# kowallus/mbgc

Measured on AMD Instinct MI355X. Metric: input Gbases/s (compress hot path, -m1: match-finding + stream emission), higher is better.
Workload: dtype u8

## Files before the change

include/mbgc_swsem.h:

```cpp
#ifndef MBGC_SWSEM_H
#define MBGC_SWSEM_H
#include <stddef.h>
#include <stdint.h>

#ifdef __cplusplus
extern "C" {
#endif

#define SWSEM_NO_LOCK   UINT64_MAX
#define SWSEM_SKIPPED   UINT64_MAX

#define SWSEM_OK         0
#define SWSEM_EINVAL    -1
#define SWSEM_ENOMEM    -2
#define SWSEM_EHIP      -3
#define SWSEM_ELOCK     -4
#define SWSEM_ENODEV    -5

typedef struct swsem swsem_t;

typedef struct {
    uint64_t posSrcText, length, posDestText;
} swsem_match_t;

const char *swsem_last_error(void);
int swsem_device_count(void);
int swsem_device_numa_node(int device);

int swsem_create(swsem_t **out, uint64_t maxRefLength, int L, int k1, int k2, int skipMargin, int device);
void swsem_destroy(swsem_t *h);
int swsem_set_stream(swsem_t *h, void *hip_stream);
int swsem_synchronize(swsem_t *h);

void swsem_disable_sliding_window(swsem_t *h);
void swsem_set_sliding_window_size(swsem_t *h, int factor);
void swsem_disable_circular_buffer(swsem_t *h);
uint64_t swsem_get_ref_length(const swsem_t *h);
uint64_t swsem_get_loading_position(const swsem_t *h);
uint64_t swsem_get_loaded_ref_length(const swsem_t *h);
uint64_t swsem_get_max_ref_length(const swsem_t *h);
uint64_t swsem_get_sliding_window_size(const swsem_t *h);
uint64_t swsem_get_dropped_bytes(const swsem_t *h);
void swsem_set_position(swsem_t *h, uint64_t refPos, int reachedRefLengthCount);
uint64_t swsem_acquire_lock(swsem_t *h);
int swsem_release_lock(swsem_t *h, uint64_t lockValue);
int swsem_get_K(const swsem_t *h);
uint32_t swsem_get_hash_size(const swsem_t *h);

int swsem_load_ref(swsem_t *h, const uint8_t *text, uint64_t len, int loadRC, int addSep, int sep);
int swsem_load_ref_dev(swsem_t *h, const uint8_t *text_dev, uint64_t len, int loadRC, int addSep, int sep);
int swsem_load_separator(swsem_t *h, int sep);
int swsem_finalize_targets(swsem_t *h, int n, const uint8_t *const *ext_dev, const uint64_t *ext_len, int addSep, int sep,
                           int lazySeparator, const uint64_t *lockPos, uint64_t *loadedAfter);
int swsem_revcomp_dev(swsem_t *h, const uint8_t *src_dev, uint64_t n, uint8_t *dst_dev);

int swsem_match(swsem_t *h, const uint8_t *query, uint64_t len, uint32_t minMatchLength, uint64_t lockPos,
                const swsem_match_t **matches, uint64_t *nmatches);

int swsem_match_batch_dev(swsem_t *h, const uint8_t *queries_dev, const uint64_t *offsets, int n,
                          uint32_t minMatchLength, const uint64_t *lockPos);
int swsem_batch_counts(swsem_t *h, uint64_t *nmatches );
int swsem_batch_matches(swsem_t *h, int contig, swsem_match_t *out, uint64_t cap);
int swsem_batch_fingerprint(swsem_t *h, uint64_t *fp, uint64_t *total_matches, uint64_t *total_length);

typedef struct {
    int enableExtensionsWithMismatches;
    int mismatchesWithExclusion;
    int lazyDecompressionSupport;
    int enable40bitReference;
    int frugal64bitLenEncoding;
    int gapDepthOffsetEncoding;
    int gapDepthMismatchesEncoding;
    uint64_t gapBreakingMatchMinLength;
    int mmsMatchBonus, mmsMismatchPenalty, mmsMismatchesScoreThreshold, mmsMismatchesInitialScore;
    int allowedTargetsOutrunForDissimilarContigs;
    uint64_t minimalLengthForDissimilarContigs;
    int unmatchedFractionFactorTweakForDissimilarContigs;
} swsem_emit_params_t;
void swsem_emit_params_default(swsem_emit_params_t *p, int mode );

enum { SWSEM_LIT = 0, SWSEM_OFF = 1, SWSEM_OFF5 = 2, SWSEM_LEN = 3, SWSEM_GAP = 4, SWSEM_FLAGS = 5, SWSEM_NSTREAMS = 6 };

typedef struct {
    const uint8_t *data[SWSEM_NSTREAMS];
    uint64_t size[SWSEM_NSTREAMS];
    uint64_t unmatchedChars;
    uint64_t extensionsMatchedChars, extensionsMismatches, totalMatched, removedGapBreakingMatches;
    uint64_t nmatches;
} swsem_streams_t;

int swsem_emit(swsem_t *h, const swsem_emit_params_t *p, int contig, uint64_t lockPos,
               int unmatchedFractionFactor, int64_t processedTargetsCount, int64_t targetIdx,
               const uint64_t *refExtLoadedPos, uint64_t nLoaded, swsem_streams_t *out);

int swsem_emit_batch(swsem_t *h, const swsem_emit_params_t *p, int n, const int *contigIdx, const uint64_t *lockPos,
                     const int *unmatchedFractionFactor, const int64_t *processedTargetsCount, const int64_t *targetIdx,
                     const uint64_t *refExtLoadedPos, uint64_t nLoaded);
int swsem_emit_batch_begin(swsem_t *h, const swsem_emit_params_t *p, int n, const int *contigIdx, const uint64_t *lockPos,
                           const int *unmatchedFractionFactor, const int64_t *processedTargetsCount, const int64_t *targetIdx,
                           const uint64_t *refExtLoadedPos, uint64_t nLoaded);
typedef struct {
    int ntargets;
    const uint8_t *const *ext_dev; const uint64_t *ext_len;
    int addSep, sep, lazySeparator;
    const uint64_t *lockPos;
    uint64_t *loadedAfter;
    const uint8_t *predExt, *predRC;
    int factor, rcFactor;
    uint32_t *gate_dev;
    int (*exchange)(void *ctx, int phase, void *gate_dev, void *stream);
    void *exchange_ctx;
    int veto;
} swsem_spec_finalize_t;
int swsem_emit_batch_begin_spec(swsem_t *h, const swsem_emit_params_t *p, int n, const int *contigIdx, const uint64_t *lockPos,
                                const int *unmatchedFractionFactor, const int64_t *processedTargetsCount, const int64_t *targetIdx,
                                const uint64_t *refExtLoadedPos, uint64_t nLoaded, const swsem_spec_finalize_t *spec, int *applied);
int swsem_emit_batch_end(swsem_t *h);
int swsem_emit_select(swsem_t *h, int previous);
int swsem_emit_result(swsem_t *h, int k, swsem_streams_t *out);
void swsem_emit_set_host_copy(swsem_t *h, int on);
int swsem_emit_unmatched(swsem_t *h, uint64_t *unmatched );
int swsem_emit_pack_dev(swsem_t *h, uint8_t *dst_dev, uint64_t cap, uint64_t *sizes, uint64_t *total);
int swsem_emit_pack_dev_on(swsem_t *h, uint8_t *dst_dev, uint64_t cap, void *stream);
int swsem_emit_counters(swsem_t *h, uint64_t *out );

typedef struct {
    const uint8_t *stream_dev[SWSEM_NSTREAMS];
    uint64_t size[SWSEM_NSTREAMS];
    uint64_t refLockPos;
    uint8_t *dest_dev;
    uint64_t destCap;
} swsem_decode_job_t;
int swsem_decode_contigs_dev(swsem_t *h, const swsem_emit_params_t *p, int n, const swsem_decode_job_t *jobs,
                             uint64_t *destLen, int64_t *unmatched);
int swsem_emit_verify(swsem_t *h, int *nbad, int *firstBad, uint64_t *firstDiff);

int swsem_create_decoder(swsem_t **out, uint64_t maxRefLength, int device);
typedef struct {
    uint64_t cur[SWSEM_NSTREAMS], end[SWSEM_NSTREAMS];
    uint32_t firstTarget, nTargets, checkEnd, pad;
} swsem_chain_start_t;
typedef struct {
    uint64_t destLen; int64_t unmatched;
    uint64_t cur[SWSEM_NSTREAMS];
    uint64_t litEnd, minSrc, maxSrcEnd, nrec;
} swsem_chain_contig_t;
int swsem_decode_plan_chain_dev(swsem_t *h, const swsem_emit_params_t *p, const uint8_t *const stream_dev[SWSEM_NSTREAMS],
                                const uint64_t size[SWSEM_NSTREAMS], int nstarts, const swsem_chain_start_t *starts, int ntargets,
                                const uint32_t *seqCount, const uint64_t *lockPos, uint64_t ncontigs, swsem_chain_contig_t *out,
                                int *firstBadChain);
int swsem_decode_fill_range_dev(swsem_t *h, uint64_t c0, uint64_t c1, uint8_t *dest_dev, const uint64_t *destOff, uint64_t *nbad);
enum { SWSEM_SEG_RC = 1, SWSEM_SEG_FROM_REF = 2, SWSEM_SEG_BYTE = 4 };
typedef struct { uint64_t src, dst, len; uint32_t flags, pad; } swsem_load_seg_t;
int swsem_decode_load_dev(swsem_t *h, const uint8_t *src_dev, int n, const swsem_load_seg_t *segs);

int swsem_dev_malloc(swsem_t *h, uint64_t bytes, void **out_dev);
int swsem_dev_free(swsem_t *h, void *p_dev);
int swsem_dev_upload(swsem_t *h, void *dst_dev, const void *src_host, uint64_t bytes);
int swsem_dev_download(swsem_t *h, void *dst_host, const void *src_dev, uint64_t bytes);
int swsem_dev_copy(swsem_t *h, void *dst_dev, const void *src_dev, uint64_t bytes);

int swsem_debug_copy_ref(swsem_t *h, uint64_t from, uint64_t n, uint8_t *out);
int swsem_debug_write_ref(swsem_t *h, uint64_t from, uint64_t n, const uint8_t *in);
int swsem_debug_copy_ht(swsem_t *h, uint32_t *out );
enum { SWSEM_K_LOAD = 0, SWSEM_K_INSERT = 1, SWSEM_K_PROBE = 2 , SWSEM_K_EMIT2 = 3, SWSEM_K_RESOLVE = 4,
       SWSEM_K_STITCH = 5, SWSEM_K_EMIT = 6, SWSEM_K_COUNT = 7 };
int swsem_debug_emit_stats(swsem_t *h, uint64_t out[8]);
int swsem_debug_block_times(swsem_t *h, uint64_t *out , uint64_t cap, uint64_t *nblocks);
int swsem_profile_enable(swsem_t *h, int on);
int swsem_profile_get(swsem_t *h, double ms[SWSEM_K_COUNT], uint64_t launches[SWSEM_K_COUNT]);
int swsem_batch_stats(swsem_t *h, uint64_t stats[6]);

#ifdef __cplusplus
}
#endif
#endif
```

mbgc_amd/binding.py:

```python
import ctypes as C
import os

import numpy as np

HERE = os.path.dirname(os.path.abspath(__file__))
LIB_PATH = os.environ.get("MBGC_HIP_LIB", os.path.join(HERE, "libmbgc_hip.so"))
NO_LOCK = 2 ** 64 - 1
SKIPPED = 2 ** 64 - 1
STREAM_NAMES = ("literals", "mapOff", "mapOff5th", "mapLen", "gapDelta", "flags")
KERNEL_FAMILIES = ("load", "insert", "probe", "emit2", "resolve", "stitch", "emit")

EXPORTS = """swsem_last_error swsem_device_count swsem_device_numa_node swsem_create swsem_destroy swsem_set_stream swsem_synchronize
swsem_disable_sliding_window swsem_set_sliding_window_size swsem_disable_circular_buffer swsem_get_ref_length
swsem_get_loading_position swsem_get_loaded_ref_length swsem_get_max_ref_length swsem_get_sliding_window_size swsem_get_dropped_bytes swsem_set_position
swsem_acquire_lock swsem_release_lock swsem_get_K swsem_get_hash_size swsem_load_ref swsem_load_ref_dev
swsem_load_separator swsem_finalize_targets swsem_revcomp_dev swsem_match swsem_match_batch_dev swsem_batch_counts swsem_batch_matches
swsem_batch_fingerprint swsem_emit_params_default swsem_emit swsem_emit_batch swsem_emit_batch_begin swsem_emit_batch_begin_spec swsem_emit_batch_end swsem_emit_select swsem_emit_result swsem_emit_set_host_copy swsem_emit_unmatched swsem_emit_pack_dev swsem_emit_pack_dev_on swsem_emit_counters swsem_debug_copy_ref swsem_debug_write_ref swsem_debug_copy_ht swsem_debug_emit_stats
swsem_profile_enable swsem_profile_get swsem_batch_stats swsem_dev_malloc swsem_dev_free swsem_dev_upload swsem_dev_download swsem_dev_copy swsem_decode_contigs_dev swsem_emit_verify
swsem_create_decoder swsem_decode_plan_chain_dev swsem_decode_fill_range_dev swsem_decode_load_dev""".split()


class SpecFinalize(C.Structure):
    _fields_ = [("ntargets", C.c_int), ("ext_dev", C.c_void_p), ("ext_len", C.POINTER(C.c_uint64)), ("addSep", C.c_int), ("sep", C.c_int),
                ("lazySeparator", C.c_int), ("lockPos", C.POINTER(C.c_uint64)), ("loadedAfter", C.POINTER(C.c_uint64)),
                ("predExt", C.c_void_p), ("predRC", C.c_void_p), ("factor", C.c_int), ("rcFactor", C.c_int),
                ("gate_dev", C.c_void_p), ("exchange", C.c_void_p), ("exchange_ctx", C.c_void_p), ("veto", C.c_int)]


SPEC_EXCHANGE = C.CFUNCTYPE(C.c_int, C.c_void_p, C.c_int, C.c_void_p, C.c_void_p)


class SwsemError(RuntimeError):
    pass


class EmitParams(C.Structure):
    _fields_ = [("enableExtensionsWithMismatches", C.c_int), ("mismatchesWithExclusion", C.c_int),
                ("lazyDecompressionSupport", C.c_int), ("enable40bitReference", C.c_int),
                ("frugal64bitLenEncoding", C.c_int), ("gapDepthOffsetEncoding", C.c_int),
                ("gapDepthMismatchesEncoding", C.c_int), ("gapBreakingMatchMinLength", C.c_uint64),
                ("mmsMatchBonus", C.c_int), ("mmsMismatchPenalty", C.c_int),
                ("mmsMismatchesScoreThreshold", C.c_int), ("mmsMismatchesInitialScore", C.c_int),
                ("allowedTargetsOutrunForDissimilarContigs", C.c_int),
                ("minimalLengthForDissimilarContigs", C.c_uint64),
                ("unmatchedFractionFactorTweakForDissimilarContigs", C.c_int)]


class DecodeJob(C.Structure):
    _fields_ = [("stream_dev", C.c_void_p * 6), ("size", C.c_uint64 * 6), ("refLockPos", C.c_uint64), ("dest_dev", C.c_void_p),
                ("destCap", C.c_uint64)]


class ChainStart(C.Structure):
    _fields_ = [("cur", C.c_uint64 * 6), ("end", C.c_uint64 * 6), ("firstTarget", C.c_uint32), ("nTargets", C.c_uint32),
                ("checkEnd", C.c_uint32), ("pad", C.c_uint32)]


class ChainContig(C.Structure):
    _fields_ = [("destLen", C.c_uint64), ("unmatched", C.c_int64), ("cur", C.c_uint64 * 6), ("litEnd", C.c_uint64),
                ("minSrc", C.c_uint64), ("maxSrcEnd", C.c_uint64), ("nrec", C.c_uint64)]


class LoadSeg(C.Structure):
    _fields_ = [("src", C.c_uint64), ("dst", C.c_uint64), ("len", C.c_uint64), ("flags", C.c_uint32), ("pad", C.c_uint32)]


SEG_RC, SEG_FROM_REF, SEG_BYTE = 1, 2, 4


class Streams(C.Structure):
    _fields_ = [("data", C.POINTER(C.c_uint8) * 6), ("size", C.c_uint64 * 6), ("unmatchedChars", C.c_uint64),
                ("extensionsMatchedChars", C.c_uint64), ("extensionsMismatches", C.c_uint64),
                ("totalMatched", C.c_uint64), ("removedGapBreakingMatches", C.c_uint64), ("nmatches", C.c_uint64)]


_lib = None


def lib():
    global _lib
    if _lib is None:
        if not os.path.exists(LIB_PATH):
            raise SwsemError("%s is missing: run `python -c 'import __graft_entry__ as g; g.build()'`" % LIB_PATH)
        try:
            import torch
        except ImportError:
            pass
        L = C.CDLL(LIB_PATH)
        u64, vp, ci, pu64 = C.c_uint64, C.c_void_p, C.c_int, C.POINTER(C.c_uint64)
        L.swsem_last_error.restype = C.c_char_p
        L.swsem_create.argtypes = [C.POINTER(vp), u64, ci, ci, ci, ci, ci]
        L.swsem_destroy.argtypes = [vp]
        L.swsem_set_stream.argtypes = [vp, vp]
        L.swsem_synchronize.argtypes = [vp]
        for n in ("swsem_disable_sliding_window", "swsem_disable_circular_buffer"):
            getattr(L, n).argtypes = [vp]
            getattr(L, n).restype = None
        L.swsem_set_sliding_window_size.argtypes = [vp, ci]
        L.swsem_set_sliding_window_size.restype = None
        for n in ("swsem_get_ref_length", "swsem_get_loading_position", "swsem_get_loaded_ref_length",
                  "swsem_get_max_ref_length", "swsem_get_sliding_window_size", "swsem_get_dropped_bytes", "swsem_acquire_lock"):
            getattr(L, n).restype = u64
            getattr(L, n).argtypes = [vp]
        L.swsem_set_position.argtypes = [vp, u64, ci]
        L.swsem_set_position.restype = None
        L.swsem_release_lock.argtypes = [vp, u64]
        L.swsem_get_K.argtypes = [vp]
        L.swsem_get_hash_size.restype = C.c_uint32
        L.swsem_get_hash_size.argtypes = [vp]
        L.swsem_load_ref.argtypes = [vp, vp, u64, ci, ci, ci]
        L.swsem_load_ref_dev.argtypes = [vp, vp, u64, ci, ci, ci]
        L.swsem_load_separator.argtypes = [vp, ci]
        L.swsem_revcomp_dev.argtypes = [vp, vp, u64, vp]
        L.swsem_finalize_targets.argtypes = [vp, ci, vp, pu64, ci, ci, ci, pu64, pu64]
        L.swsem_match.argtypes = [vp, vp, u64, C.c_uint32, u64, C.POINTER(vp), pu64]
        L.swsem_match_batch_dev.argtypes = [vp, vp, pu64, ci, C.c_uint32, pu64]
        L.swsem_batch_counts.argtypes = [vp, pu64]
        L.swsem_batch_matches.argtypes = [vp, ci, vp, u64]
        L.swsem_batch_fingerprint.argtypes = [vp, pu64, pu64, pu64]
        L.swsem_emit_params_default.argtypes = [C.POINTER(EmitParams), ci]
        L.swsem_emit_params_default.restype = None
        L.swsem_emit.argtypes = [vp, C.POINTER(EmitParams), ci, u64, ci, C.c_int64, C.c_int64, vp, u64,
                                 C.POINTER(Streams)]
        L.swsem_emit_batch.argtypes = [vp, C.POINTER(EmitParams), ci, vp, vp, vp, vp, vp, vp, u64]
        L.swsem_emit_batch_begin.argtypes = L.swsem_emit_batch.argtypes
        L.swsem_emit_batch_end.argtypes = [vp]
        L.swsem_emit_batch_begin_spec.argtypes = L.swsem_emit_batch.argtypes + [C.POINTER(SpecFinalize), C.POINTER(C.c_int)]
        L.swsem_emit_select.argtypes = [vp, ci]
        L.swsem_emit_result.argtypes = [vp, ci, C.POINTER(Streams)]
        L.swsem_emit_set_host_copy.argtypes = [vp, ci]
        L.swsem_emit_set_host_copy.restype = None
        L.swsem_emit_pack_dev.argtypes = [vp, vp, u64, pu64, pu64]
        L.swsem_emit_pack_dev_on.argtypes = [vp, vp, u64, vp]
        L.swsem_emit_counters.argtypes = [vp, pu64]
        L.swsem_emit_unmatched.argtypes = [vp, pu64]
        L.swsem_emit_verify.argtypes = [vp, C.POINTER(ci), C.POINTER(ci), pu64]
        L.swsem_decode_contigs_dev.argtypes = [vp, C.POINTER(EmitParams), ci, vp, pu64, C.POINTER(C.c_int64)]
        L.swsem_create_decoder.argtypes = [C.POINTER(vp), u64, ci]
        L.swsem_decode_plan_chain_dev.argtypes = [vp, C.POINTER(EmitParams), C.POINTER(vp), pu64, ci, C.POINTER(ChainStart), ci,
                                                  C.POINTER(C.c_uint32), pu64, u64, C.POINTER(ChainContig), C.POINTER(ci)]
        L.swsem_decode_fill_range_dev.argtypes = [vp, u64, u64, vp, pu64, pu64]
        L.swsem_decode_load_dev.argtypes = [vp, vp, ci, C.POINTER(LoadSeg)]
        L.swsem_debug_copy_ref.argtypes = [vp, u64, u64, vp]
        L.swsem_debug_write_ref.argtypes = [vp, u64, u64, vp]
        L.swsem_debug_copy_ht.argtypes = [vp, vp]
        L.swsem_profile_enable.argtypes = [vp, ci]
        L.swsem_profile_get.argtypes = [vp, C.POINTER(C.c_double), pu64]
        L.swsem_batch_stats.argtypes = [vp, pu64]
        _lib = L
    return _lib


def _chk(rc):
    if rc != 0:
        raise SwsemError("swsem error %d: %s" % (rc, lib().swsem_last_error().decode()))


def _bytes_ptr(a):
    a = np.ascontiguousarray(a, dtype=np.uint8)
    return a, a.ctypes.data_as(C.c_void_p)


def emit_params(mode=1, **over):
    p = EmitParams()
    lib().swsem_emit_params_default(C.byref(p), mode)
    for k, v in over.items():
        setattr(p, k, v)
    return p


class SlidingWindowSparseEMMatcher:

    def __init__(self, max_ref_len, L=32, k1=16, k2=1, skip_margin=16, device=0):
        self.h = C.c_void_p()
        _chk(lib().swsem_create(C.byref(self.h), max_ref_len, L, k1, k2, skip_margin, device))

    def close(self):
        if getattr(self, "h", None):
            lib().swsem_destroy(self.h)
            self.h = None

    def __del__(self):
        self.close()

    def disable_sliding_window(self): lib().swsem_disable_sliding_window(self.h)
    def set_sliding_window_size(self, f): lib().swsem_set_sliding_window_size(self.h, f)
    def disable_circular_buffer(self): lib().swsem_disable_circular_buffer(self.h)
    def ref_length(self): return lib().swsem_get_ref_length(self.h)
    def loading_position(self): return lib().swsem_get_loading_position(self.h)
    def loaded_ref_length(self): return lib().swsem_get_loaded_ref_length(self.h)
    def max_ref_length(self): return lib().swsem_get_max_ref_length(self.h)
    def sliding_window_size(self): return lib().swsem_get_sliding_window_size(self.h)
    def dropped_bytes(self): return lib().swsem_get_dropped_bytes(self.h)

    def emit_stats(self):
        out = (C.c_uint64 * 8)()
        lib().swsem_debug_emit_stats.argtypes = [C.c_void_p, C.POINTER(C.c_uint64)]
        _chk(lib().swsem_debug_emit_stats(self.h, out))
        return {"foreign_boundary_steps": int(out[4]), "blocks_not_accepted": int(out[5]), "groups_replayed": int(out[6]),
                "blocks_given_up": int(out[7])}
    def set_position(self, pos, laps): lib().swsem_set_position(self.h, pos, laps)
    def acquire_lock(self): return lib().swsem_acquire_lock(self.h)
    def release_lock(self, v): _chk(lib().swsem_release_lock(self.h, v)); return 0
    def hash_size(self): return lib().swsem_get_hash_size(self.h)
    def K(self): return lib().swsem_get_K(self.h)
    def set_stream(self, stream_ptr): _chk(lib().swsem_set_stream(self.h, stream_ptr))
    def synchronize(self): _chk(lib().swsem_synchronize(self.h))

    def load_ref(self, text, load_rc=False, add_sep=True, sep=0):
        a, p = _bytes_ptr(text)
        _chk(lib().swsem_load_ref(self.h, p, a.size, int(load_rc), int(add_sep), sep))

    def load_ref_dev(self, dev_ptr, n, load_rc=False, add_sep=True, sep=0):
        _chk(lib().swsem_load_ref_dev(self.h, dev_ptr, n, int(load_rc), int(add_sep), sep))

    def load_separator(self, sep=0): _chk(lib().swsem_load_separator(self.h, sep))

    def finalize_targets(self, ext_ptrs, ext_lens, locks, lazy=True, add_sep=True, sep=0):
        n = len(ext_lens)
        ptrs = (C.c_void_p * n)(*[int(p) for p in ext_ptrs])
        lens = np.ascontiguousarray(ext_lens, dtype=np.uint64)
        lk = np.ascontiguousarray(locks, dtype=np.uint64)
        out = np.zeros(n, dtype=np.uint64)
        P = C.POINTER(C.c_uint64)
        _chk(lib().swsem_finalize_targets(self.h, n, ptrs, lens.ctypes.data_as(P), int(add_sep), sep, int(lazy),
                                          lk.ctypes.data_as(P), out.ctypes.data_as(P)))
        return out
    def revcomp_dev(self, src_ptr, n, dst_ptr): _chk(lib().swsem_revcomp_dev(self.h, src_ptr, n, dst_ptr))

    def match(self, q, min_len=32, lock=NO_LOCK):
        a, p = _bytes_ptr(q)
        out, n = C.c_void_p(), C.c_uint64()
        _chk(lib().swsem_match(self.h, p, a.size, min_len, lock, C.byref(out), C.byref(n)))
        if n.value == 0:
            return np.zeros((0, 3), dtype=np.uint64)
        return np.ctypeslib.as_array(C.cast(out, C.POINTER(C.c_uint64)), shape=(n.value, 3)).copy()

    def match_batch_dev(self, dev_ptr, offsets, min_len=32, locks=None):
        offs = np.ascontiguousarray(offsets, dtype=np.uint64)
        n = offs.size - 1
        lk = None
        if locks is not None:
            lk = np.ascontiguousarray(locks, dtype=np.uint64)
            assert lk.size == n
        _chk(lib().swsem_match_batch_dev(self.h, dev_ptr, offs.ctypes.data_as(C.POINTER(C.c_uint64)), n, min_len,
                                         lk.ctypes.data_as(C.POINTER(C.c_uint64)) if lk is not None else None))
        self._batch_n = n

    def batch_counts(self):
        out = np.zeros(self._batch_n, dtype=np.uint64)
        _chk(lib().swsem_batch_counts(self.h, out.ctypes.data_as(C.POINTER(C.c_uint64))))
        return out

    def batch_matches(self, contig, count):
        out = np.zeros((int(count), 3), dtype=np.uint64)
        _chk(lib().swsem_batch_matches(self.h, contig, out.ctypes.data_as(C.c_void_p), int(count)))
        return out

    def batch_fingerprint(self):
        fp, tot, ln = C.c_uint64(), C.c_uint64(), C.c_uint64()
        _chk(lib().swsem_batch_fingerprint(self.h, C.byref(fp), C.byref(tot), C.byref(ln)))
        return fp.value, tot.value, ln.value

    def batch_stats(self):
        s = (C.c_uint64 * 6)()
        _chk(lib().swsem_batch_stats(self.h, s))
        return dict(zip(("bases", "probes", "hits", "matches", "matched_len", "replayed_blocks"), s))

    def emit(self, params, contig=0, lock=NO_LOCK, factor=128, processed=0, target_idx=0, loaded=None):
        ld = np.ascontiguousarray(loaded if loaded is not None else [0], dtype=np.uint64)
        st = Streams()
        _chk(lib().swsem_emit(self.h, C.byref(params), contig, lock, factor, processed, target_idx,
                              ld.ctypes.data_as(C.c_void_p), ld.size, C.byref(st)))
        streams = {}
        for i, name in enumerate(STREAM_NAMES):
            n = st.size[i]
            streams[name] = bytes(np.ctypeslib.as_array(st.data[i], shape=(n,))) if n else b""
        return st.unmatchedChars, streams, st

    def emit_batch(self, params, contigs=None, locks=None, factors=None, processed=None, target_idx=None, loaded=None, n=None,
                   _entry="swsem_emit_batch"):
        def arr(x, dt):
            return None if x is None else np.ascontiguousarray(x, dtype=dt)
        ci, lk, fa = arr(contigs, np.int32), arr(locks, np.uint64), arr(factors, np.int32)
        pr, ti = arr(processed, np.int64), arr(target_idx, np.int64)
        ld = np.ascontiguousarray(loaded if loaded is not None else [0], dtype=np.uint64)
        cnt = n if n is not None else (ci.size if ci is not None else self._batch_n)
        ptr = lambda a: None if a is None else a.ctypes.data_as(C.c_void_p)
        _chk(getattr(lib(), _entry)(self.h, C.byref(params), cnt, ptr(ci), ptr(lk), ptr(fa), ptr(pr), ptr(ti), ptr(ld), ld.size))
        return cnt

    def emit_batch_begin(self, *a, **k):
        return self.emit_batch(*a, _entry="swsem_emit_batch_begin", **k)

    def emit_batch_end(self): _chk(lib().swsem_emit_batch_end(self.h))

    def emit_batch_begin_spec(self, params, locks, factors, processed, target_idx, loaded, n, ext_ptrs, ext_lens, target_locks,
                              pred_ext, pred_rc, factor, rc_factor, lazy=True, add_sep=True, sep=0, gate=0, reduce=None,
                              verdict=None, veto=False):
        u64, P = np.uint64, C.POINTER(C.c_uint64)
        lk, fa = np.ascontiguousarray(locks, dtype=u64), np.ascontiguousarray(factors, dtype=np.int32)
        pr, ti = np.ascontiguousarray(processed, dtype=np.int64), np.ascontiguousarray(target_idx, dtype=np.int64)
        ld = np.ascontiguousarray(loaded if loaded is not None else [0], dtype=u64)
        nt = len(ext_lens)
        ptrs = (C.c_void_p * nt)(*[int(x) for x in ext_ptrs])
        lens = np.ascontiguousarray(ext_lens, dtype=u64)
        tl = np.ascontiguousarray(target_locks, dtype=u64)
        after = np.zeros(nt, dtype=u64)
        pe, prc = np.ascontiguousarray(pred_ext, dtype=np.uint8), np.ascontiguousarray(pred_rc, dtype=np.uint8)
        sp = SpecFinalize(nt, C.cast(ptrs, C.c_void_p), lens.ctypes.data_as(P), int(add_sep), sep, int(lazy), tl.ctypes.data_as(P),
                          after.ctypes.data_as(P), pe.ctypes.data_as(C.c_void_p), prc.ctypes.data_as(C.c_void_p), int(factor), int(rc_factor))
        failure = []
        if reduce is not None:
            def _cb(ctx, phase, gate_dev, stream):
                try:
                    if phase == 0:
                        reduce(stream)
                        return 0
                    return int(verdict())
                except BaseException as e:
                    failure.append(e)
                    return -1
            cb = SPEC_EXCHANGE(_cb)
            sp.gate_dev, sp.exchange, sp.veto = int(gate), C.cast(cb, C.c_void_p), int(veto)
        applied = C.c_int()
        vp = lambda a: a.ctypes.data_as(C.c_void_p)
        rc = lib().swsem_emit_batch_begin_spec(self.h, C.byref(params), n, None, vp(lk), vp(fa), vp(pr), vp(ti), vp(ld), ld.size,
                                               C.byref(sp), C.byref(applied))
        if failure:
            raise failure[0]
        _chk(rc)
        return bool(applied.value), after
    def emit_select(self, previous): _chk(lib().swsem_emit_select(self.h, int(previous)))

    def emit_set_host_copy(self, on): lib().swsem_emit_set_host_copy(self.h, int(on))

    def emit_verify(self):
        nbad, first, diff = C.c_int(), C.c_int(), C.c_uint64()
        _chk(lib().swsem_emit_verify(self.h, C.byref(nbad), C.byref(first), C.byref(diff)))
        return nbad.value, first.value, diff.value

    def decode_contigs_dev(self, params, jobs):
        n = len(jobs)
        arr = (DecodeJob * n)()
        for k, (streams, lock, dest, cap) in enumerate(jobs):
            for st, (ptr, size) in enumerate(streams):
                arr[k].stream_dev[st] = ptr
                arr[k].size[st] = size
            arr[k].refLockPos, arr[k].dest_dev, arr[k].destCap = lock, dest, cap
        dl = np.zeros(n, dtype=np.uint64)
        un = np.zeros(n, dtype=np.int64)
        _chk(lib().swsem_decode_contigs_dev(self.h, C.byref(params), n, C.cast(arr, C.c_void_p), dl.ctypes.data_as(C.POINTER(C.c_uint64)),
                                            un.ctypes.data_as(C.POINTER(C.c_int64))))
        return dl, un

    def emit_pack_sizes(self, n):
        sizes = np.zeros(n * 6, dtype=np.uint64)
        tot = C.c_uint64()
        _chk(lib().swsem_emit_pack_dev(self.h, None, 0, sizes.ctypes.data_as(C.POINTER(C.c_uint64)), C.byref(tot)))
        return sizes.reshape(n, 6), tot.value

    def emit_pack_dev(self, dst_ptr, cap, stream=None):
        if stream is not None:
            _chk(lib().swsem_emit_pack_dev_on(self.h, dst_ptr, cap, C.c_void_p(stream)))
            return None
        tot = C.c_uint64()
        _chk(lib().swsem_emit_pack_dev(self.h, dst_ptr, cap, None, C.byref(tot)))
        return tot.value

    def emit_unmatched(self, n):
        out = np.zeros(n, dtype=np.uint64)
        _chk(lib().swsem_emit_unmatched(self.h, out.ctypes.data_as(C.POINTER(C.c_uint64))))
        return out

    def emit_result(self, k):
        st = Streams()
        _chk(lib().swsem_emit_result(self.h, k, C.byref(st)))
        streams = {}
        for i, name in enumerate(STREAM_NAMES):
            sz = st.size[i]
            streams[name] = bytes(np.ctypeslib.as_array(st.data[i], shape=(sz,))) if sz else b""
        return st.unmatchedChars, streams, st

    def ref(self, n=None, start=0):
        n = self.ref_length() if n is None else n
        out = np.zeros(n, dtype=np.uint8)
        _chk(lib().swsem_debug_copy_ref(self.h, start, n, out.ctypes.data_as(C.c_void_p)))
        return out

    def write_ref(self, start, data):
        a = np.ascontiguousarray(data, dtype=np.uint8)
        _chk(lib().swsem_debug_write_ref(self.h, start, a.size, a.ctypes.data_as(C.c_void_p)))

    def ht(self):
        out = np.zeros(self.hash_size(), dtype=np.uint32)
        _chk(lib().swsem_debug_copy_ht(self.h, out.ctypes.data_as(C.c_void_p)))
        return out

    def profile_enable(self, on=True): _chk(lib().swsem_profile_enable(self.h, int(on)))

    def profile_get(self):
        ms = (C.c_double * 7)()
        n = (C.c_uint64 * 7)()
        _chk(lib().swsem_profile_get(self.h, ms, n))
        return {KERNEL_FAMILIES[i]: (ms[i], n[i]) for i in range(7)}


class Decoder(SlidingWindowSparseEMMatcher):

    def __init__(self, max_ref_len, device=0):
        self.h = C.c_void_p()
        _chk(lib().swsem_create_decoder(C.byref(self.h), max_ref_len, device))

    def plan_chain(self, params, streams, starts, seq_counts, locks):
        ptrs = (C.c_void_p * 6)(*[int(p) for p, _ in streams])
        sizes = (C.c_uint64 * 6)(*[int(n) for _, n in streams])
        st = (ChainStart * len(starts))()
        for k, (cur, end, t0, nt, chk) in enumerate(starts):
            for i in range(6):
                st[k].cur[i], st[k].end[i] = int(cur[i]), int(end[i])
            st[k].firstTarget, st[k].nTargets, st[k].checkEnd = t0, nt, int(chk)
        sc = np.ascontiguousarray(seq_counts, dtype=np.uint32)
        lk = np.ascontiguousarray(locks, dtype=np.uint64)
        n = int(sc.sum())
        out = (ChainContig * max(n, 1))()
        bad = C.c_int(-1)
        _chk(lib().swsem_decode_plan_chain_dev(self.h, C.byref(params), ptrs, sizes, len(starts), st, sc.size,
                                               sc.ctypes.data_as(C.POINTER(C.c_uint32)), lk.ctypes.data_as(C.POINTER(C.c_uint64)), n, out, C.byref(bad)))
        return list(out[:n]), bad.value

    def fill_range(self, c0, c1, dest_ptr, dest_off):
        off = np.ascontiguousarray(dest_off, dtype=np.uint64)
        nbad = C.c_uint64()
        _chk(lib().swsem_decode_fill_range_dev(self.h, c0, c1, dest_ptr, off.ctypes.data_as(C.POINTER(C.c_uint64)), C.byref(nbad)))
        return nbad.value

    def load_segments(self, src_ptr, segs):
        arr = (LoadSeg * max(len(segs), 1))()
        for k, (src, dst, ln, fl) in enumerate(segs):
            arr[k].src, arr[k].dst, arr[k].len, arr[k].flags = int(src), int(dst), int(ln), int(fl)
        _chk(lib().swsem_decode_load_dev(self.h, src_ptr, len(segs), arr))
```

mbgc_amd/csrc/swsem_kernels.hip:

```cpp
#include "swsem_device.h"

namespace swk {


__global__ void __launch_bounds__(256) k_load_rc(const uint8_t *__restrict__ src, uint8_t *__restrict__ dst,
                                                 uint64_t n, const uint8_t *__restrict__ lut) {
    __shared__ uint8_t slut[256];
    slut[threadIdx.x] = lut[threadIdx.x];
    __syncthreads();
    const uint64_t stride = (uint64_t) gridDim.x * blockDim.x * 4;
    for (uint64_t d = ((uint64_t) blockIdx.x * blockDim.x + threadIdx.x) * 4; d < n; d += stride) {
        const uint64_t m = n - d < 4 ? n - d : 4;
#pragma unroll
        for (uint64_t k = 0; k < 4; k++)
            if (k < m) dst[d + k] = slut[src[n - 1 - d - k]];
    }
}

__global__ void k_set_byte(uint8_t *p, uint8_t v) { *p = v; }
__global__ void k_touch() {}
__global__ void __launch_bounds__(256) k_hog(unsigned long long ticks) {
    const unsigned long long t0 = __builtin_amdgcn_s_memrealtime();
    while (__builtin_amdgcn_s_memrealtime() - t0 < ticks) __builtin_amdgcn_s_sleep(8);
}

struct CopyPiece { uint64_t dst; const uint8_t *src; uint64_t len; };
struct BytePiece { uint64_t off, val; };
__global__ void __launch_bounds__(256) k_copy_multi(uint8_t *__restrict__ ref, const CopyPiece *__restrict__ pieces,
                                                    const uint64_t *__restrict__ first, int np, const uint32_t *__restrict__ gate) {
    if (gate && *gate == 0) return;
    for (uint64_t blk = blockIdx.x; blk < first[np]; blk += gridDim.x) {
        int lo = 0, hi = np - 1;
        while (lo < hi) {
            const int mid = (lo + hi + 1) / 2;
            if (first[mid] <= blk) lo = mid; else hi = mid - 1;
        }
        const CopyPiece pc = pieces[lo];
        const uint64_t o = (blk - first[lo]) * 4096 + 16 * (uint64_t) threadIdx.x;
        if (o >= pc.len) continue;
        uint8_t *d = ref + pc.dst + o;
        const uint8_t *s = pc.src + o;
        if (o + 16 <= pc.len) {
            uint4 t;
            memcpy(&t, s, 16);
            memcpy(d, &t, 16);
        } else
            for (uint64_t k = 0; k < pc.len - o; k++) d[k] = s[k];
    }
}
__global__ void __launch_bounds__(256) k_upload(uint8_t *__restrict__ dst, const uint8_t *__restrict__ src, uint64_t n) {
    const uint64_t o = 16 * ((uint64_t) blockIdx.x * 256 + threadIdx.x);
    if (o + 16 <= n) {
        uint4 t;
        memcpy(&t, src + o, 16);
        memcpy(dst + o, &t, 16);
    } else
        for (uint64_t k = o; k < n; k++) dst[k] = src[k];
}
struct CopySegs { static constexpr int MAX = 8; uint8_t *dst[MAX]; const uint8_t *src[MAX]; uint64_t bytes[MAX]; uint32_t first[MAX + 1]; int n; };
__global__ void __launch_bounds__(256) k_copy_segs(CopySegs sg) {
    int k = 0;
    while (k + 1 < sg.n && blockIdx.x >= sg.first[k + 1]) k++;
    const uint64_t o = 16 * ((uint64_t) (blockIdx.x - sg.first[k]) * 256 + threadIdx.x), n = sg.bytes[k];
    uint8_t *dst = sg.dst[k];
    const uint8_t *src = sg.src[k];
    if (o + 16 <= n) {
        uint4 t = make_uint4(0, 0, 0, 0);
        if (src) memcpy(&t, src + o, 16);
        memcpy(dst + o, &t, 16);
    } else
        for (uint64_t i = o; i < n; i++) dst[i] = src ? src[i] : (uint8_t) 0;
}
__global__ void k_set_bytes(uint8_t *__restrict__ ref, const BytePiece *__restrict__ b, int n, const uint32_t *__restrict__ gate) {
    if (gate && *gate == 0) return;
    for (int i = 0; i < n; i++) ref[b[i].off] = (uint8_t) b[i].val;
}


__device__ __forceinline__ uint32_t fp_at(const uint8_t *s, int nw) {
    uint32_t f = FP_SEED;
    for (int j = 0; j < nw; j++) f = fp_step(f, ld_u32(s + 4 * j));
    return f;
}

__global__ void __launch_bounds__(256) k_insert(const uint8_t *__restrict__ ref, ht_entry *__restrict__ ht,
                                                uint64_t S, uint64_t nMain, uint64_t T, uint64_t nTail, int k1,
                                                int k1ord, int K, uint32_t mask, uint32_t epoch, int fpBits,
                                                uint16_t *__restrict__ tags, uint32_t tag) {
    const uint64_t t = (uint64_t) blockIdx.x * blockDim.x + threadIdx.x;
    if (t >= nMain + nTail) return;
    const bool tail = t >= nMain;
    const uint64_t p = tail ? T + (t - nMain) * (uint64_t) k1 : S + t * (uint64_t) k1;
    if (tags && (p & ((1ull << k1ord) - 1)) == 0) tags[p >> k1ord] = (uint16_t) tag;
    const uint8_t *s = ref + p;
    uint32_t h = (uint32_t) K, f = FP_SEED;
    const int nw = K / 4;
    for (int j = 0; j < nw; j++) { const uint32_t w = ld_u32(s + 4 * j); h = hash_step(h, w, (uint32_t) j); f = fp_step(f, w); }
    const uint32_t off = (uint32_t) (p & ((1ull << k1ord) - 1));
    if (off && p >= off) f = fp_at(s - off, nw);
    const ht_entry key = ht_key(epoch + (tail ? 1u : 0u), (uint32_t) (p >> k1ord), f, fpBits);
    atomicMax(&ht[h & mask], key);
}

struct InsertPiece { uint64_t S, nMain, T, nTail; uint32_t epoch, tag; const uint8_t *src; uint64_t lo, hi; };
__device__ __forceinline__ bool insert_sample(const InsertPiece *__restrict__ pieces, const uint64_t *__restrict__ first, int np, int k1, uint64_t g,
                                              InsertPiece &pc, uint64_t &p, bool &tail) {
    int lo = 0, hi = np;
    while (hi - lo > 1) { const int mid = (lo + hi) / 2; if (first[mid] <= g) lo = mid; else hi = mid; }
    pc = pieces[lo];
    const uint64_t t = g - first[lo];
    tail = t >= pc.nMain;
    p = tail ? pc.T + (t - pc.nMain) * (uint64_t) k1 : pc.S + t * (uint64_t) k1;
    return true;
}
template<bool FROM_SRC>
__global__ void __launch_bounds__(256) k_insert_multi(const uint8_t *__restrict__ ref, ht_entry *__restrict__ ht,
                                                      const InsertPiece *__restrict__ pieces, const uint64_t *__restrict__ first,
                                                      int np, int k1, int k1ord, int K, uint32_t mask, int fpBits,
                                                      const uint32_t *__restrict__ gate, uint16_t *__restrict__ tags) {
    if (gate && *gate == 0) return;
    const uint64_t total = first[np];
    for (uint64_t g0 = (uint64_t) blockIdx.x * blockDim.x + threadIdx.x; g0 < total; g0 += (uint64_t) gridDim.x * blockDim.x) {
        const uint64_t g = total - 1 - g0;
        InsertPiece pc; uint64_t p; bool tail;
        insert_sample(pieces, first, np, k1, g, pc, p, tail);
        const uint8_t *s = ref + p;
        if (FROM_SRC) {
            if (!pc.src || p < pc.lo || p + (uint64_t) K > pc.hi) continue;
            s = pc.src + (p - pc.lo);
        }
        if (tags && (p & ((1ull << k1ord) - 1)) == 0) tags[p >> k1ord] = (uint16_t) pc.tag;
        uint32_t h = (uint32_t) K, f = FP_SEED;
        const int nw = K / 4;
        for (int j = 0; j < nw; j++) { const uint32_t w = ld_u32(s + 4 * j); h = hash_step(h, w, (uint32_t) j); f = fp_step(f, w); }
        const uint32_t off = (uint32_t) (p & ((1ull << k1ord) - 1));
        if (off && p >= off && (!FROM_SRC || p - off >= pc.lo)) f = fp_at(s - off, nw);
        const ht_entry key = ht_key(pc.epoch + (tail ? 1u : 0u), (uint32_t) (p >> k1ord), f, fpBits);
        const ht_entry seen = ht[h & mask];
        if (seen >= key) continue;
        atomicMax(&ht[h & mask], key);
    }
}
__global__ void k_mark_stale(const uint8_t *__restrict__ ref, ht_entry *__restrict__ ht, uint64_t p, int K, int k1ord, uint32_t mask, int fpBits,
                             uint16_t *__restrict__ tags) {
    if (tags) tags[p >> k1ord] = 0;
    uint32_t h = (uint32_t) K;
    for (int j = 0; j < K / 4; j++) h = hash_step(h, ld_u32(ref + p + 4 * j), (uint32_t) j);
    const ht_entry e = ht[h & mask];
    if ((uint32_t) (e >> fpBits) == (uint32_t) (p >> k1ord) && e != 0)
        ht[h & mask] = e & ((((ht_entry) 1) << (32 + fpBits)) - 1);
}

__global__ void __launch_bounds__(256) k_ht_low_words(const ht_entry *__restrict__ ht, uint32_t *__restrict__ out, uint64_t n, int fpBits) {
    const uint64_t i = (uint64_t) blockIdx.x * blockDim.x + threadIdx.x;
    if (i < n) out[i] = (uint32_t) (ht[i] >> fpBits);
}

struct Chain {
    int32_t scan;
    int32_t minTouched;
    int32_t minKeep;
    int32_t visited;
    uint32_t cands;
    bool emitted;
#ifdef SWSEM_DIAG_PHASES
    uint64_t tRefill, tVisit, tLcp;
    uint32_t nRefill, nLcp;
#endif
};
#ifdef SWSEM_DIAG_PHASES
__device__ unsigned long long g_diag[8];
#endif

constexpr int RING = 64;

__device__ __forceinline__ uint32_t rl32(uint32_t x, int lane) { return (uint32_t) __builtin_amdgcn_readlane((int) x, lane); }
__device__ __forceinline__ uint32_t rfl32(uint32_t x) { return (uint32_t) __builtin_amdgcn_readfirstlane((int) x); }
__device__ __forceinline__ uint64_t rfl64(uint64_t x) { return ((uint64_t) rfl32((uint32_t) (x >> 32)) << 32) | rfl32((uint32_t) x); }
constexpr int OVERLAP_MAX = 1024;
constexpr int SNAP = 4;

struct __attribute__((aligned(16))) Row {
    uint64_t posSrc, len, posDest;
    int64_t scanAfter;
};
__device__ __forceinline__ void put_row(Match *dst, const Match &m, int64_t) { *dst = m; }
__device__ __forceinline__ void put_row(Row *dst, const Match &m, int64_t scan) {
    Row r;
    r.posSrc = m.posSrc; r.len = m.len; r.posDest = m.posDest; r.scanAfter = scan;
    *dst = r;
}

template <class R>
struct ArrayStack {
    R *st;
    uint2 *ring;
    int32_t sp, ringLow;
    __device__ __forceinline__ int size() const { return sp; }
    __device__ __forceinline__ void get(int idx, int32_t &posDest, int32_t &len) {
        if (idx >= ringLow) {
            const uint2 e = ring[idx & (RING - 1)];
            posDest = (int32_t) rfl32(e.x); len = (int32_t) rfl32(e.y);
        } else {
            posDest = (int32_t) rfl32((uint32_t) st[idx].posDest); len = (int32_t) rfl32((uint32_t) st[idx].len);
        }
    }
    __device__ __forceinline__ void truncate_push(int keep, const Match &m, int32_t scanAfter) {
        sp = keep;
        if ((threadIdx.x & (WAVE - 1)) == 0) put_row(st + sp, m, scanAfter);
        ring[sp & (RING - 1)] = make_uint2((uint32_t) m.posDest, (uint32_t) m.len);
        if (sp - (RING - 1) > ringLow) ringLow = sp - (RING - 1);
        if (ringLow > sp) ringLow = sp;
        sp++;
    }
};

struct VirtStack {
    Row *region;
    uint32_t cap;
    uint32_t *segStart, *keepN;
    int32_t *prev;
    int32_t segTop;
    int32_t topKeep, topPrev;
    int32_t size_;
    Row *own; int32_t ownN;
    int32_t curSeg, curLocal, curR;
    __device__ __forceinline__ int size() const { return size_; }
    __device__ __forceinline__ int keep_of(int seg) const { return seg == segTop ? topKeep : (int) rfl32(keepN[seg]); }
    __device__ __forceinline__ int prev_of(int seg) const { return seg == segTop ? topPrev : (int) rfl32((uint32_t) prev[seg]); }
    __device__ const Row *at(int idx) {
        const int below = size_ - ownN;
        if (idx >= below) return own + (idx - below);
        const int r = below - 1 - idx;
        if (curSeg < 0 || curR > r) { curSeg = segTop; curLocal = topKeep - 1; curR = 0; }
        while (curR < r) {
            const int step = r - curR < curLocal ? r - curR : curLocal;
            if (step > 0) { curLocal -= step; curR += step; }
            else { curSeg = prev_of(curSeg); curLocal = keep_of(curSeg) - 1; curR++; }
        }
        return region + (uint64_t) curSeg * cap + rfl32(segStart[curSeg]) + curLocal;
    }
    __device__ __forceinline__ void get(int idx, int32_t &posDest, int32_t &len) {
        const Row *m = at(idx);
        posDest = (int32_t) rfl32((uint32_t) m->posDest); len = (int32_t) rfl32((uint32_t) m->len);
    }
    __device__ void pop_segments(int p) {
        const bool l0 = (threadIdx.x & (WAVE - 1)) == 0;
        while (p > 0) {
            const int take = topKeep < p ? topKeep : p;
            topKeep -= take;
            p -= take;
            if (topKeep == 0) {
                if (l0) keepN[segTop] = 0;
                const int nt = topPrev;
                if (nt >= 0) { topKeep = (int) rfl32(keepN[nt]); topPrev = (int) rfl32((uint32_t) prev[nt]); }
                segTop = nt;
            }
        }
        curSeg = -1;
    }
    __device__ void truncate_push(int keep, const Match &m, int32_t scanAfter) {
        int p = size_ - keep;
        const int t = p < ownN ? p : ownN;
        ownN -= t; p -= t;
        if (p > 0) pop_segments(p);
        if ((threadIdx.x & (WAVE - 1)) == 0) put_row(own + ownN, m, scanAfter);
        ownN++;
        size_ = keep + 1;
    }
    __device__ void push_segment(int b, uint32_t start, uint32_t n) {
        if (n == 0) return;
        if ((threadIdx.x & (WAVE - 1)) == 0) {
            if (segTop >= 0) keepN[segTop] = (uint32_t) topKeep;
            segStart[b] = start; prev[b] = segTop;
        }
        topPrev = segTop;
        segTop = b;
        topKeep = (int32_t) n;
        size_ += (int32_t) n;
        curSeg = -1;
    }
    __device__ void flush() { if (segTop >= 0 && (threadIdx.x & (WAVE - 1)) == 0) keepN[segTop] = (uint32_t) topKeep; }
};

__device__ uint32_t wave_lcp_fwd(const uint8_t *a, const uint8_t *b, uint32_t n, uint32_t limit, int steps, bool &more) {
    const uint32_t lane = threadIdx.x & (WAVE - 1);
    more = false;
    while (n < limit) {
        const uint32_t off = n + 4 * lane;
        uint32_t eq = 4;
        bool stop = false;
        if (off + 4 <= limit) {
            const uint32_t x = ld_u32(a + off) ^ ld_u32(b + off);
            if (x) { eq = (uint32_t) (__builtin_ctz(x) >> 3); stop = true; }
        } else {
            eq = 0; stop = true;
            if (off < limit) {
                const uint32_t avail = limit - off;
                while (eq < avail && a[off + eq] == b[off + eq]) eq++;
            }
        }
        const unsigned long long bal = __ballot(stop);
        if (bal) {
            const int l = __builtin_ctzll(bal);
            return n + 4 * (uint32_t) l + rl32(eq, l);
        }
        n += 4 * WAVE;
        if (steps && --steps == 0 && n < limit) { more = true; return n; }
    }
    return limit;
}
__device__ uint32_t wave_lcp_bwd(const uint8_t *a, const uint8_t *b, uint32_t n, uint32_t limit, int steps, bool &more) {
    const uint32_t lane = threadIdx.x & (WAVE - 1);
    more = false;
    while (n < limit) {
        const uint32_t off = n + 4 * lane;
        uint32_t eq = 4;
        bool stop = false;
        if (off + 4 <= limit) {
            const uint32_t x = ld_u32(a - off - 4) ^ ld_u32(b - off - 4);
            if (x) { eq = (uint32_t) (__builtin_clz(x) >> 3); stop = true; }
        } else {
            eq = 0; stop = true;
            if (off < limit) {
                const uint32_t avail = limit - off;
                while (eq < avail && a[-(int64_t) (off + eq) - 1] == b[-(int64_t) (off + eq) - 1]) eq++;
            }
        }
        const unsigned long long bal = __ballot(stop);
        if (bal) {
            const int l = __builtin_ctzll(bal);
            return n + 4 * (uint32_t) l + rl32(eq, l);
        }
        n += 4 * WAVE;
        if (steps && --steps == 0 && n < limit) { more = true; return n; }
    }
    return limit;
}

template <class Stack>
__device__ bool process_hit(const RefView &v, const Contig &cg, const uint8_t *q, Stack &stk, Chain &ch,
                            uint64_t c, int32_t i, int32_t ell, int32_t rext, int32_t loDist, uint32_t flags) {
    const int32_t K = v.K;
    uint64_t lo = 0, hi = 0;
    if (flags) window_ok(v, cg.lock, c, lo, hi);
    auto need_ell = [&](int32_t x) {
        if ((flags & HIT_CAPL) && x > ell) {
            const uint64_t d = c - lo;
            const uint32_t jmax = (uint64_t) i < d ? (uint32_t) i : (uint32_t) d;
            bool more;
#ifdef SWSEM_DIAG_PHASES
            const uint64_t dl0 = __builtin_amdgcn_s_memtime();
#endif
            ell = (int32_t) wave_lcp_bwd(v.ref + c, q + i, (uint32_t) ell, jmax, 0, more);
#ifdef SWSEM_DIAG_PHASES
            ch.tLcp += __builtin_amdgcn_s_memtime() - dl0; ch.nLcp++;
#endif
            flags &= ~HIT_CAPL;
        }
    };
    int32_t s = 0;
    int keep = stk.size();
    bool brokeOut = false;
    while (keep-- > 0) {
        int32_t mPos, mLen;
        stk.get(keep, mPos, mLen);
        const int32_t mEnd = mPos + mLen;
        if (mEnd < i - s) {
            const int32_t g = mEnd;
            need_ell((loDist < i - g + 1 ? loDist : i - g + 1) - 1);
            int32_t t = loDist < i - g + 1 ? loDist : i - g + 1;
            if (ell + 1 < t) t = ell + 1;
            if (t > s) s = t;
            if (i - s > g - 1) { brokeOut = true; break; }
            s -= 1;
        }
        const int32_t d = (i - s) - mPos;
        bool fail = (loDist - s < d) || (mLen > OVERLAP_MATCH_MAX_LENGTH);
        if (!fail) {
            need_ell(s + d);
            fail = ell < s + d;
        }
        if (fail) { s += 1; brokeOut = true; break; }
        s += d;
    }
    if (!brokeOut) keep = -1;
    if (keep < ch.minTouched) ch.minTouched = keep;
    ch.visited++;
    if (keep < 0) {
        need_ell((loDist < i + 1 ? loDist : i + 1) - 1);
        int32_t t = loDist < i + 1 ? loDist : i + 1;
        if (ell + 1 < t) t = ell + 1;
        if (t > s) s = t;
    } else {
        int32_t mPos, mLen;
        stk.get(keep, mPos, mLen);
        const int32_t overlap = (mPos + mLen) - (i - s + 1);
        if (overlap > 0) s -= overlap;
    }
    ++keep;
    if (K + rext + s > (int32_t) v.minLen || (flags & HIT_CAPR)) {
        if (flags & HIT_CAPR) {
            const uint64_t a = hi - (c + K);
            const uint32_t b = (uint32_t) cg.n - (uint32_t) (i + K);
            bool more;
#ifdef SWSEM_DIAG_PHASES
            const uint64_t dl0 = __builtin_amdgcn_s_memtime();
#endif
            rext = (int32_t) wave_lcp_fwd(v.ref + c + K, q + i + K, (uint32_t) rext, a < b ? (uint32_t) a : b, 0, more);
#ifdef SWSEM_DIAG_PHASES
            ch.tLcp += __builtin_amdgcn_s_memtime() - dl0; ch.nLcp++;
#endif
            flags &= ~HIT_CAPR;
        }
        if (K + rext + s > (int32_t) v.minLen) {
            Match m;
            m.posSrc = c - (uint64_t) (int64_t) (s - 1);
            m.len = (uint64_t) (uint32_t) (K + rext + s - 1);
            m.posDest = (uint64_t) (uint32_t) (i - s + 1);
            int32_t skip = K + rext;
            skip -= skip > v.skipMargin ? v.skipMargin : skip;
            ch.scan = skip ? i + skip : i + 1;
            stk.truncate_push(keep, m, ch.scan);
            if (keep < ch.minKeep) ch.minKeep = keep;
            ch.emitted = true;
            return true;
        }
    }
    ch.scan = i + 1;
    return false;
}

constexpr int LEFTW = 64;

template <class Stack>
__device__ void visit(const RefView &v, const Contig &cg, const uint8_t *q, Stack &stk, Chain &ch, int32_t i, uint32_t val) {
    const int32_t lane = (int32_t) (threadIdx.x & (WAVE - 1));
    ch.cands++;
    const uint64_t c = (uint64_t) val << v.k1ord;
    uint64_t lo, hi;
    window_ok(v, cg.lock, c, lo, hi);
    const int32_t K = v.K;
    const uint8_t *r0 = v.ref + c, *q0 = q + i;
    const uint64_t ra = hi - (c + K);
    const uint32_t rb = (uint32_t) cg.n - (uint32_t) (i + K);
    const int32_t limR = (int32_t) (ra < rb ? (uint32_t) ra : rb);
    const uint64_t d = c - lo;
    const int32_t limL = (uint64_t) i < d ? i : (int32_t) d;
    constexpr int LL = LEFTW / 4;
    const int32_t rel = 4 * lane - LEFTW;
    const bool full = lane < LL ? -rel <= limL : rel + 4 <= K + limR;
    uint32_t x = 0;
#ifdef SWSEM_DIAG_PHASES
    const uint64_t dv0 = __builtin_amdgcn_s_memtime();
#endif
    if (full) x = ld_u32(r0 + rel) ^ ld_u32(q0 + rel);
    const unsigned long long stopAll = __ballot(!full || x != 0);
#ifdef SWSEM_DIAG_PHASES
    ch.tVisit += __builtin_amdgcn_s_memtime() - dv0;
#endif
    const unsigned long long fwd = stopAll >> LL;
    if (fwd & ((1ull << (K / 4)) - 1)) { ch.scan = i + 1; return; }
    const unsigned long long fullAll = __ballot(full);
    int32_t rext = 4 * (WAVE - LL) - K;
    const bool capR = fwd == 0;
    if (!capR) {
        const int l = LL + __builtin_ctzll(fwd);
        rext = 4 * (l - LL) - K;
        if ((fullAll >> l) & 1) rext += __builtin_ctz(rl32(x, l)) >> 3;
        else while (rext < limR && r0[K + rext] == q0[K + rext]) rext++;
    }
    const uint32_t bwd = (uint32_t) stopAll & ((1u << LL) - 1);
    int32_t ell = LEFTW;
    const bool capL = bwd == 0;
    if (!capL) {
        const int l = 31 - __builtin_clz(bwd);
        ell = 4 * (LL - 1 - l);
        if ((fullAll >> l) & 1) ell += __builtin_clz(rl32(x, l)) >> 3;
        else while (ell < limL && r0[-ell - 1] == q0[-ell - 1]) ell++;
    }
    process_hit(v, cg, q, stk, ch, c, i, ell, rext, (int32_t) (d > 0x7FFFFFFFull ? 0x7FFFFFFFull : d),
                (capL ? HIT_CAPL : 0u) | (capR ? HIT_CAPR : 0u));
}

struct NoStop { __device__ __forceinline__ bool operator()() { return false; } };

#ifndef SWSEM_WL
#define SWSEM_WL 32
#endif
constexpr int WL = SWSEM_WL;
#ifndef SWSEM_RESOLVE_SGPRS
#define SWSEM_RESOLVE_SGPRS 88
#endif
#ifndef SWSEM_RESOLVE_WAVES
#define SWSEM_RESOLVE_WAVES 7
#endif
constexpr int RESOLVE_WAVES_PER_SIMD = SWSEM_RESOLVE_WAVES;
__device__ __forceinline__ uint32_t window_hash(const RefView &v, const uint8_t *q, int32_t s, int32_t cnt, int32_t lane, uint32_t &fpHash) {
    const uintptr_t A = (uintptr_t) (q + s);
    const uint32_t sh = (uint32_t) (A & 3);
    const uint32_t *A0 = (const uint32_t *) (A & ~(uintptr_t) 3);
    const uint32_t ndw = (sh + (uint32_t) cnt + (uint32_t) v.K - 1u + 3u) >> 2;
    const uint32_t a = (uint32_t) lane < ndw ? A0[lane] : 0u;
    const uint32_t o = sh + (uint32_t) lane, wi = o >> 2, sft = o & 3u;
    const int nw = v.K / 4;
    uint32_t h = (uint32_t) v.K, f = FP_SEED;
    uint32_t lo = (uint32_t) __builtin_amdgcn_ds_bpermute((int) (wi << 2), (int) a);
    for (int x = 0; x < nw; x++) {
        const uint32_t hi = (uint32_t) __builtin_amdgcn_ds_bpermute((int) ((wi + (uint32_t) x + 1u) << 2), (int) a);
        const uint32_t w = __builtin_amdgcn_alignbyte(hi, lo, sft);
        h = hash_step(h, w, (uint32_t) x);
        f = fp_step(f, w);
        lo = hi;
    }
    fpHash = f;
    return h;
}

template <bool LAPS, class Stack, class Stop = NoStop>
__device__ void run_chain_lazy(const RefView &v, const Contig &cg, const uint8_t *q,
                               int32_t p0, int32_t p1, Stack &stk, Chain &ch, Stop stop = Stop()) {
    const int32_t lane = (int32_t) (threadIdx.x & (WAVE - 1));
    int32_t wb = -0x40000000;
    uint32_t w = 0;
    unsigned long long m = 0;
    uint32_t prioTick = 0;
    while (true) {
        const int32_t s = ch.scan > p0 ? ch.scan : p0;
        if (s >= p1) break;
        ch.scan = s;
        if (s < wb || s >= wb + WL) {
            switch ((prioTick++ + blockIdx.x) & 3u) {
                case 0: __builtin_amdgcn_s_setprio(0); break;
                case 1: __builtin_amdgcn_s_setprio(1); break;
                case 2: __builtin_amdgcn_s_setprio(2); break;
                default: __builtin_amdgcn_s_setprio(3); break;
            }
            wb = s;
#ifdef SWSEM_DIAG_PHASES
            const uint64_t dt0 = __builtin_amdgcn_s_memtime();
#endif
            const int32_t pos = s + lane;
            uint32_t e = 0;
            uint32_t hf;
            const uint32_t hv = window_hash(v, q, s, p1 - s < WL ? p1 - s : WL, lane, hf);
            if (lane < WL && pos < p1) {
                const ht_entry hte = v.ht[hv & v.mask];
                e = ht_value<LAPS>(v, hte, hf);
                if (e != 0) {
                    uint64_t lo, hi;
                    if (!window_ok(v, cg.lock, (uint64_t) e << v.k1ord, lo, hi)) e = 0;
                    else if (stale_settled<LAPS>(v, hte, e)) e = 0;
                }
            }
            w = e;
            m = __ballot(w != 0);
#ifdef SWSEM_DIAG_PHASES
            ch.tRefill += __builtin_amdgcn_s_memtime() - dt0; ch.nRefill++;
#endif
        }
        const unsigned long long mk = m & ~((1ull << (s - wb)) - 1);
        if (!mk) { ch.scan = wb + WL < p1 ? wb + WL : p1; continue; }
        const int l = __builtin_ctzll(mk);
        visit(v, cg, q, stk, ch, wb + l, rl32(w, l));
        if (stop()) return;
    }
}


template <bool LAPS, class Stack, class Stop = NoStop>
__device__ __forceinline__ void chain_run(const RefView &v, const Contig &cg, const uint8_t *q, int32_t p0, int32_t p1, Stack &stk, Chain &ch,
                                          Stop stop = Stop()) {
    run_chain_lazy<LAPS>(v, cg, q, p0, p1, stk, ch, stop);
}

template <bool LAPS>
__global__ void __launch_bounds__(WAVE) k_resolve_seq(RefView v, const uint8_t *__restrict__ qbuf,
                                                      const Contig *__restrict__ contigs,
                                                      Match *__restrict__ matches, uint32_t *__restrict__ matchCount) {
    __shared__ uint2 ring[RING];
    const Contig cg = contigs[blockIdx.x];
    Chain ch;
    ch.scan = 0; ch.minTouched = 0; ch.minKeep = 0; ch.visited = 0; ch.cands = 0; ch.emitted = false;
    ArrayStack<Match> stk;
    stk.st = matches + cg.matchBase; stk.ring = ring; stk.sp = 0; stk.ringLow = 0;
    const int32_t npos = cg.n >= (uint64_t) v.K ? (int32_t) (cg.n - v.K + 1) : 0;
    chain_run<LAPS>(v, cg, qbuf + cg.qoff, 0, npos, stk, ch);
    if (threadIdx.x == 0) matchCount[blockIdx.x] = (uint32_t) stk.sp;
}

struct __attribute__((aligned(16))) BlockRec {
    int64_t scanB;
    int64_t scanF;
    int32_t spB, spF;
    int32_t minTouched;
    int32_t minKeep;
    uint64_t cycles;
    uint32_t visits, emits;
    Match bTop[SNAP];
    Match fTop[SNAP];
};

__device__ __forceinline__ void snapshot_top(const Row *st, int sp, Match *out) {
#pragma unroll
    for (int j = 0; j < SNAP; j++) {
        if (j < sp) { out[j].posSrc = st[sp - 1 - j].posSrc; out[j].len = st[sp - 1 - j].len; out[j].posDest = st[sp - 1 - j].posDest; }
        else { out[j].posSrc = 0; out[j].len = 0; out[j].posDest = 0; }
    }
}

template <bool LAPS>
__global__ void __launch_bounds__(WAVE) __attribute__((amdgpu_num_sgpr(SWSEM_RESOLVE_SGPRS))) k_resolve_blocks(RefView v, const uint8_t *__restrict__ qbuf,
                                                         const Contig *__restrict__ contigs,
                                                         const uint32_t *__restrict__ rbContig,
                                                         const uint32_t *__restrict__ order,
                                                         Row *__restrict__ regions, uint32_t cap, uint32_t rb,
                                                         BlockRec *__restrict__ recs, uint32_t overlap) {
    __shared__ uint2 ring[RING];
    const uint32_t g = order[blockIdx.x];
    if (g == 0xFFFFFFFFu) return;
    const Contig cg = contigs[rbContig[g]];
    const uint32_t b = g - cg.rb0;
    const int32_t npos = cg.n >= (uint64_t) v.K ? (int32_t) (cg.n - v.K + 1) : 0;
    const int32_t w0 = (int32_t) (b * rb * RBU);
    const int32_t w1 = w0 + (int32_t) (rb * RBU) < npos ? w0 + (int32_t) (rb * RBU) : npos;
    Chain ch;
    const int32_t warm0 = w0 > (int32_t) overlap ? w0 - (int32_t) overlap : 0;
    ch.scan = b ? warm0 : 0; ch.minTouched = 0x7fffffff; ch.minKeep = 0x7fffffff; ch.visited = 0; ch.cands = 0; ch.emitted = false;
#ifdef SWSEM_DIAG_PHASES
    ch.tRefill = ch.tVisit = ch.tLcp = 0; ch.nRefill = ch.nLcp = 0;
#endif
    const uint64_t tstart = __builtin_amdgcn_s_memtime();
#ifdef SWSEM_DIAG_T0
    const uint64_t rt0 = __builtin_amdgcn_s_memrealtime();
#endif
    ArrayStack<Row> stk;
    stk.st = regions + (uint64_t) g * cap; stk.ring = ring; stk.sp = 0; stk.ringLow = 0;
    const uint8_t *q = qbuf + cg.qoff;
    if (b) chain_run<LAPS>(v, cg, q, warm0, w0, stk, ch);
    BlockRec r;
    r.scanB = ch.scan > w0 ? ch.scan : w0;
    r.spB = stk.sp;
    __builtin_amdgcn_s_waitcnt(0);
    snapshot_top(stk.st, stk.sp, r.bTop);
    ch.minTouched = 0x7fffffff; ch.minKeep = stk.sp; ch.visited = 0;
    chain_run<LAPS>(v, cg, q, w0, w1, stk, ch);
    r.scanF = ch.scan;
    r.spF = stk.sp;
    r.minTouched = ch.visited ? ch.minTouched : 0x7fffffff;
    r.minKeep = ch.minKeep < r.spB ? ch.minKeep : r.spB;
    __builtin_amdgcn_s_waitcnt(0);
    snapshot_top(stk.st, stk.sp, r.fTop);
    r.cycles = __builtin_amdgcn_s_memtime() - tstart;
    r.visits = ch.cands; r.emits = (uint32_t) (stk.sp);
#ifdef SWSEM_DIAG_T0
    r.visits = (uint32_t) rt0;
    r.emits = (uint32_t) __builtin_amdgcn_s_memrealtime();
#endif
    if (threadIdx.x == 0) recs[g] = r;
#ifdef SWSEM_DIAG_PHASES
    if (threadIdx.x == 0) {
        atomicAdd(&g_diag[0], (unsigned long long) r.cycles); atomicAdd(&g_diag[1], (unsigned long long) ch.tRefill);
        atomicAdd(&g_diag[2], (unsigned long long) ch.tVisit); atomicAdd(&g_diag[3], (unsigned long long) ch.nRefill);
        atomicAdd(&g_diag[4], (unsigned long long) ch.cands); atomicAdd(&g_diag[5], (unsigned long long) ch.tLcp);
        atomicAdd(&g_diag[6], (unsigned long long) ch.nLcp); atomicAdd(&g_diag[7], 1ull);
    }
#endif
}

__device__ __forceinline__ bool same_match(const Match &a, const Match &b) {
    return a.posSrc == b.posSrc && a.len == b.len && a.posDest == b.posDest;
}

struct __attribute__((aligned(16))) FastRec {
    int32_t scanF;
    int32_t minKeep;
    int32_t npush;
    int32_t popB;
};
__global__ void __launch_bounds__(256) k_stitch_pre(const Contig *__restrict__ contigs, const uint32_t *__restrict__ rbContig,
                                                    const BlockRec *__restrict__ recs, uint32_t rb, uint32_t nblocks,
                                                    FastRec *__restrict__ fast) {
    const uint32_t g = blockIdx.x * blockDim.x + threadIdx.x;
    if (g >= nblocks) return;
    const Contig cg = contigs[rbContig[g]];
    const uint32_t b = g - cg.rb0;
    const BlockRec &cur = recs[g];
    FastRec f;
    f.scanF = (int32_t) cur.scanF; f.minKeep = cur.minKeep; f.npush = cur.spF - cur.minKeep; f.popB = -1;
    const bool visited = cur.minTouched != 0x7fffffff;
    if (b == 0) {
        if (visited) f.popB = 0;
    } else if (visited && cur.minTouched >= 0) {
        const BlockRec &prv = recs[g - 1];
        const int32_t span = (int32_t) (rb * RBU), w0 = (int32_t) b * span;
        const int32_t pScanF = (int32_t) prv.scanF;
        const int cmp = cur.spB - cur.minTouched;
        const int prevPush = prv.spF - prv.minKeep;
        bool ok = prv.minTouched != 0x7fffffff && pScanF < w0 + span && (pScanF > w0 ? pScanF : w0) == (int32_t) cur.scanB &&
                  cmp >= 0 && cmp <= SNAP && cmp <= prevPush;
        for (int j = 0; ok && j < cmp; j++)
            ok = cur.bTop[j].posSrc == prv.fTop[j].posSrc && cur.bTop[j].len == prv.fTop[j].len && cur.bTop[j].posDest == prv.fTop[j].posDest;
        if (ok) f.popB = cur.spB - cur.minKeep;
    }
    fast[g] = f;
}

template <bool LAPS>
__global__ void __launch_bounds__(WAVE) k_stitch(RefView v, const uint8_t *__restrict__ qbuf,
                                                 const Contig *__restrict__ contigs,
                                                 Row *__restrict__ regions, Row *__restrict__ replayArea,
                                                 uint32_t cap, uint32_t rb, const BlockRec *__restrict__ recs,
                                                 const FastRec *__restrict__ fast,
                                                 uint32_t *__restrict__ segStart, uint32_t *__restrict__ keepN,
                                                 int32_t *__restrict__ prev, uint32_t *__restrict__ dstOff,
                                                 uint32_t *__restrict__ matchCount,
                                                 unsigned long long *__restrict__ stats) {
    const Contig cg = contigs[blockIdx.x];
    const uint32_t lane = threadIdx.x;
    const uint8_t *q = qbuf + cg.qoff;
    VirtStack vs;
    vs.region = regions + (uint64_t) cg.rb0 * cap; vs.cap = cap;
    vs.segStart = segStart + cg.rb0; vs.keepN = keepN + cg.rb0; vs.prev = prev + cg.rb0;
    vs.segTop = -1; vs.topKeep = 0; vs.topPrev = -1; vs.size_ = 0; vs.own = nullptr; vs.ownN = 0; vs.curSeg = -1; vs.curLocal = 0; vs.curR = 0;
    for (uint32_t b = lane; b < cg.nrb; b += WAVE) { vs.keepN[b] = 0; vs.segStart[b] = 0; }
    __builtin_amdgcn_s_waitcnt(0);
    int32_t scanT = 0;
    constexpr int TW = 3 * SNAP;
    __shared__ uint64_t ptop[TW];
    int known = 0;
    uint32_t replayed = 0, nFast = 0, nSlow = 0, nSkip = 0;
    const BlockRec *rc = recs + cg.rb0;
    const int32_t span = (int32_t) (rb * RBU);
    const int32_t npos = cg.n >= (uint64_t) v.K ? (int32_t) (cg.n - v.K + 1) : 0;
    __shared__ uint4 srec[sizeof(BlockRec) / 16];
    bool prevPlain = true;
    uint4 fr = make_uint4(0, 0, 0, 0);
    for (uint32_t b = 0; b < cg.nrb; b++) {
        if ((b & (WAVE - 1)) == 0) fr = b + lane < cg.nrb ? ((const uint4 *) (fast + cg.rb0))[b + lane] : make_uint4(0, 0, 0, 0xFFFFFFFFu);
        const int32_t w0 = (int32_t) b * span;
        if (scanT >= w0 + span) { prevPlain = false; nSkip++; continue; }
        const int fl = (int) (b & (WAVE - 1));
        const int32_t fPop = (int32_t) rl32(fr.w, fl);
        if (prevPlain && fPop >= 0) {
            const unsigned long long fastMask = __ballot((int32_t) fr.w >= 0);
            const unsigned long long rest = ~(fastMask >> fl);
            const int L = rest ? __builtin_ctzll(rest) : WAVE - fl;
            const bool inRun = (int) lane >= fl && (int) lane < fl + L;
            const int32_t myPop = inRun ? (int32_t) fr.w : 0, myPush = inRun ? (int32_t) fr.z : 0;
            int32_t nextPop = __shfl_down(myPop, 1);
            if ((int) lane + 1 >= fl + L) nextPop = 0;
            if (fPop > 0) vs.pop_segments(fPop);
            const unsigned long long segMask = __ballot(inRun && myPush > 0);
            int32_t delta = myPush - myPop;
            for (int d = WAVE / 2; d > 0; d >>= 1) delta += __shfl_xor(delta, d);
            vs.size_ += delta;
            if (segMask) {
                if (lane == 0 && vs.segTop >= 0) vs.keepN[vs.segTop] = (uint32_t) vs.topKeep;
                const int32_t b0 = (int32_t) b - fl;
                const unsigned long long below = segMask & ((1ull << lane) - 1ull);
                const int32_t pv = below ? b0 + (63 - __builtin_clzll(below)) : vs.segTop;
                const int32_t keepMine = myPush - nextPop;
                if (inRun && myPush > 0) {
                    vs.segStart[b0 + (int32_t) lane] = (uint32_t) fr.y;
                    vs.prev[b0 + (int32_t) lane] = pv;
                    vs.keepN[b0 + (int32_t) lane] = (uint32_t) keepMine;
                }
                const int top = 63 - __builtin_clzll(segMask);
                vs.segTop = b0 + top;
                vs.topKeep = (int32_t) rl32((uint32_t) keepMine, top);
                vs.topPrev = (int32_t) rl32((uint32_t) pv, top);
                vs.curSeg = -1;
            }
            scanT = (int32_t) rl32(fr.x, fl + L - 1);
            known = 0;
            b += (uint32_t) (L - 1);
            nFast += (uint32_t) L;
            continue;
        }
        nSlow++;
        {
            const uint4 *src = (const uint4 *) (rc + b);
            for (uint32_t i = lane; i < sizeof(BlockRec) / 16; i += WAVE) srec[i] = src[i];
            __builtin_amdgcn_s_waitcnt(0);
        }
        const BlockRec *r = (const BlockRec *) srec;
        const int32_t rScanB = (int32_t) rfl32((uint32_t) r->scanB), rScanF = (int32_t) rfl32((uint32_t) r->scanF);
        const int spB = (int) rfl32((uint32_t) r->spB), spF = (int) rfl32((uint32_t) r->spF);
        const int minTouched = (int) rfl32((uint32_t) r->minTouched), minKeep = (int) rfl32((uint32_t) r->minKeep);
        const uint64_t *bw = (const uint64_t *) r->bTop, *fw = (const uint64_t *) r->fTop;
        const bool visited = minTouched != 0x7fffffff;
        bool ok;
        if (b == 0) ok = true;
        else {
            ok = (scanT > w0 ? scanT : w0) == rScanB;
            if (ok && visited) {
                const int cmp = minTouched < 0 ? spB : spB - minTouched;
                if (minTouched < 0) ok = vs.size_ == spB && spB <= SNAP;
                else ok = cmp <= SNAP && cmp <= vs.size_;
                if (ok && cmp > known) {
                    __builtin_amdgcn_s_waitcnt(0);
                    const int n = vs.size_ < SNAP ? vs.size_ : SNAP;
                    for (int j = 0; j < n; j++) {
                        const Row *m = vs.at(vs.size_ - 1 - j);
                        if (lane < 3) ptop[3 * j + lane] = ((const uint64_t *) m)[lane];
                    }
                    known = n;
                }
                if (ok) {
                    const bool diff = (int) lane < 3 * cmp && bw[lane < TW ? lane : 0] != ptop[lane < TW ? lane : 0];
                    ok = __ballot(diff) == 0;
                }
            }
        }
        if (ok) {
            if (visited || b == 0) {
                const int popB = spB - minKeep;
                const int npush = spF - minKeep;
                if (popB > 0) vs.pop_segments(popB);
                vs.size_ -= popB;
                vs.push_segment((int) b, (uint32_t) minKeep, (uint32_t) npush);
                const int keepOld = known > popB ? known - popB : 0;
                if (lane < TW) {
                    const int row = lane / 3, fld = lane % 3;
                    uint64_t x = 0;
                    if (row < npush) x = fw[lane];
                    else if (row - npush < keepOld) x = ptop[3 * (row - npush + popB) + fld];
                    ptop[lane] = x;
                }
                known = npush + keepOld < SNAP ? npush + keepOld : SNAP;
                scanT = rScanF;
                prevPlain = true;
            } else
                prevPlain = false;
        } else {
            prevPlain = false;
            Chain ch;
            ch.scan = scanT; ch.minTouched = 0x7fffffff; ch.minKeep = 0x7fffffff; ch.visited = 0; ch.cands = 0; ch.emitted = false;
            Row *own = replayArea + (uint64_t) blockIdx.x * cap;
            const Row *spec = vs.region + (uint64_t) b * cap;
            vs.own = own; vs.ownN = 0;
            int sp = minKeep < 0 ? 0 : minKeep;
            int syncAt = -1;
            auto stop = [&]() -> bool {
                if (!ch.emitted) return false;
                ch.emitted = false;
                if (vs.ownN == 0) return false;
                __builtin_amdgcn_s_waitcnt(0);
                const uint64_t ePos = rfl64(own[vs.ownN - 1].posDest), eLen = rfl64(own[vs.ownN - 1].len), eSrc = rfl64(own[vs.ownN - 1].posSrc);
                while (sp < spF && rfl64(spec[sp].posDest) < ePos) sp++;
                if (sp < spF && rfl64(spec[sp].posDest) == ePos && rfl64(spec[sp].len) == eLen && rfl64(spec[sp].posSrc) == eSrc &&
                    (int32_t) rfl32((uint32_t) spec[sp].scanAfter) == ch.scan) { syncAt = sp; return true; }
                return false;
            };
            chain_run<LAPS>(v, cg, q, w0, w0 + span < npos ? w0 + span : npos, vs, ch, stop);
            int n = vs.ownN;
            vs.size_ -= n; vs.ownN = 0; vs.own = nullptr;
            __builtin_amdgcn_s_waitcnt(0);
            Row *dst = vs.region + (uint64_t) b * cap;
            if (syncAt >= 0) {
                const int tail = spF - syncAt - 1;
                for (int k = lane; k < tail; k += WAVE) own[n + k] = spec[syncAt + 1 + k];
                n += tail;
                scanT = rScanF;
                __builtin_amdgcn_s_waitcnt(0);
            } else
                scanT = ch.scan;
            for (int k = lane; k < n; k += WAVE) dst[k] = own[k];
            __builtin_amdgcn_s_waitcnt(0);
            vs.push_segment((int) b, 0, (uint32_t) n);
            known = 0;
            replayed++;
        }
    }
    vs.flush();
    __builtin_amdgcn_s_waitcnt(0);
    uint32_t run = 0;
    for (uint32_t b0 = 0; b0 < cg.nrb; b0 += WAVE) {
        const uint32_t b = b0 + lane;
        const uint32_t k = b < cg.nrb ? vs.keepN[b] : 0;
        uint32_t x = k;
        for (int d = 1; d < WAVE; d <<= 1) {
            const uint32_t y = (uint32_t) __shfl_up((int) x, d);
            if ((int) lane >= d) x += y;
        }
        if (b < cg.nrb) dstOff[cg.rb0 + b] = run + x - k;
        run += (uint32_t) __shfl((int) x, WAVE - 1);
    }
    if (lane == 0) {
        matchCount[blockIdx.x] = run;
        atomicAdd(&stats[3], (unsigned long long) replayed);
        atomicAdd(&stats[5], (unsigned long long) nFast);
        atomicAdd(&stats[6], (unsigned long long) nSlow);
        atomicAdd(&stats[7], (unsigned long long) nSkip);
    }
}

__global__ void __launch_bounds__(WAVE) k_gather(const Contig *__restrict__ contigs, const uint32_t *__restrict__ rbContig,
                                                 const Row *__restrict__ regions, uint32_t cap,
                                                 const uint32_t *__restrict__ segStart, const uint32_t *__restrict__ keepN,
                                                 const uint32_t *__restrict__ dstOff, Match *__restrict__ matches) {
    const uint32_t g = blockIdx.x;
    const uint32_t n = keepN[g];
    if (n == 0) return;
    const Contig cg = contigs[rbContig[g]];
    const Row *src = regions + (uint64_t) g * cap + segStart[g];
    Match *dst = matches + cg.matchBase + dstOff[g];
    for (uint32_t k = threadIdx.x; k < n; k += WAVE) { Match m; m.posSrc = src[k].posSrc; m.len = src[k].len; m.posDest = src[k].posDest; dst[k] = m; }
}

__global__ void k_fingerprint(const Contig *__restrict__ contigs, int n, const Match *__restrict__ matches,
                              const uint32_t *__restrict__ matchCount, unsigned long long *out) {
    unsigned long long fp = 0xcbf29ce484222325ull, tot = 0, len = 0;
    for (int c = 0; c < n; c++) {
        const Match *m = matches + contigs[c].matchBase;
        for (uint32_t k = 0; k < matchCount[c]; k++) {
            fp ^= m[k].posSrc; fp *= 0x100000001b3ull;
            fp ^= m[k].len; fp *= 0x100000001b3ull;
            fp ^= m[k].posDest; fp *= 0x100000001b3ull;
            tot++; len += m[k].len;
        }
    }
    out[0] = fp; out[1] = tot; out[2] = len;
}

}
```

mbgc_amd/csrc/swsem_runtime.hip:

```cpp
#include "../../include/mbgc_swsem.h"
#include "swsem_kernels.hip"
#include "swsem_resolve4.hip"
#include "swsem_emit.hip"
#include "swsem_decode.hip"

#include <algorithm>
#include <cctype>
#include <chrono>
#include <mutex>
#include <cstdarg>
#include <cstdio>
#include <cstdlib>
#include <cstring>
#include <deque>
#include <string>
#include <vector>

using namespace swk;

#include "swsem_runtime_state.h"
#include "swsem_runtime_streams.h"
#include "swsem_runtime_loader.h"
#include "swsem_runtime_match.h"
#include "swsem_runtime_emit.h"
#include "swsem_runtime_decode.h"

namespace {

void init_params(swsem *h) {
    const int L = h->L;
    if (L > 110) h->K = 56;
    else if (L > 62) h->K = 44;
    else if (L > 53) h->K = 40;
    else if (L > 46) h->K = 36;
    else if (L > 42) h->K = 32;
    else if (L > 32) h->K = 28;
    else h->K = (L / 4 - 1) * 4;
    const int KmmL = (L / 4 - 1) * 4;
    if (KmmL < h->K) h->K = KmmL;
    uint8_t i = 24;
    do {
        h->hash_size = ((uint32_t) 1) << (i++);
    } while (i <= 31 && h->hash_size < h->maxRefLength / (uint64_t) h->k1);
    h->mask = h->hash_size - 1;
    h->fpBits = 10;
}

void build_lut(uint8_t *lut) {
    for (int i = 0; i < 256; i++) lut[i] = (uint8_t) i;
    lut[127] = 0;
    const char *from = "AaCcGgTtNnUuYyRrKkMmBbDdHhVvWwSs";
    const char *to = "TTGGCCAANNAARRYYMMKKVVHHDDBBSSWW";
    for (int i = 0; from[i]; i++) lut[(uint8_t) from[i]] = (uint8_t) to[i];
}

}

#define MATCHER_ONLY(h) do { if ((h)->decoder) return fail(SWSEM_EINVAL, "%s: the handle is a decoder's (swsem_create_decoder): it has no hash table", __func__); } while (0)

extern "C" {

const char *swsem_last_error(void) { return g_err.c_str(); }

int swsem_device_count(void) {
    int n = 0;
    if (hipGetDeviceCount(&n) != hipSuccess) return 0;
    return n;
}

int swsem_device_numa_node(int device) {
    char bus[64] = {0};
    int count = 0;
    if (hipGetDeviceCount(&count) != hipSuccess || device < 0 || device >= count ||
        hipDeviceGetPCIBusId(bus, (int) sizeof bus, device) != hipSuccess) {
        (void) hipGetLastError();
        return -1;
    }
    for (char *c = bus; *c; c++) *c = (char) tolower((unsigned char) *c);
    char path[160];
    snprintf(path, sizeof path, "/sys/bus/pci/devices/%s/numa_node", bus);
    FILE *f = fopen(path, "r");
    if (!f) return -1;
    int node = -1;
    if (fscanf(f, "%d", &node) != 1) node = -1;
    fclose(f);
    return node;
}

int swsem_create(swsem_t **out, uint64_t maxRefLength, int L, int k1, int k2, int skipMargin, int device) {
    *out = nullptr;
    if (k1 <= 0) return fail(SWSEM_EINVAL, "s - reference sampling step - should be a positive integer.");
    if (k2 != 1) return fail(SWSEM_EINVAL, "k2 = %d unsupported (MBGC always uses k2 = 1, MGMP_Params.h:202)", k2);
    if (L < 16) return fail(SWSEM_EINVAL, "Error: Minimal matching length too short!");
    if (maxRefLength < 64 || (maxRefLength >> __builtin_ctz((unsigned) k1)) >= (1ull << 32))
        return fail(SWSEM_EINVAL, "reference length limit %llu out of range", (unsigned long long) maxRefLength);
    int ndev = 0;
    if (hipGetDeviceCount(&ndev) != hipSuccess || ndev <= 0 || device >= ndev)
        return fail(SWSEM_ENODEV, "no HIP device %d (the HIP path has no CPU fallback)", device);
    HIPCHK(hipSetDevice(device));
    g_eventsFailed = false;
    swsem *h = new swsem();
    h->device = device;
    if (g_eventsFailed) { swsem_destroy(h); return fail(SWSEM_EHIP, "hipEventCreate failed"); }
    h->sw = read_switches();
    h->maxRefLength = maxRefLength;
    h->L = L; h->k1 = k1; h->skipMargin = skipMargin;
    h->k1ord = __builtin_ctz((unsigned) k1);
    h->ld.swEnd = maxRefLength;
    h->swSize = maxRefLength / SW_WIDTH_FACTOR;
    init_params(h);
    h->ld.samplingPos = (k1 % 2) ? REF_SHIFT : (uint64_t) k1;
    h->useTags = h->k1ord != 0 && h->sw.lapTags;
    if (hipStreamCreateWithFlags(&h->stream, hipStreamNonBlocking) != hipSuccess) { swsem_destroy(h); return fail(SWSEM_EHIP, "hipStreamCreate failed"); }
    h->ownStream = true;
    int least = 0, greatest = 0;
    if (hipDeviceGetStreamPriorityRange(&least, &greatest) == hipSuccess) { h->prioLow = least; h->prioHigh = greatest; }
    { int d = deal_streams(h); if (d) { swsem_destroy(h); return d; } }
    { hipDeviceProp_t pr; if (hipGetDeviceProperties(&pr, device) == hipSuccess && pr.multiProcessorCount > 0) h->waveSlots = (uint32_t) pr.multiProcessorCount * 4u * RESOLVE_WAVES_PER_SIMD; }
    const size_t nSlots = (size_t) ((maxRefLength + REF_SLACK) >> h->k1ord) + 2;
    if (hipMalloc((void **) &h->ref, maxRefLength + REF_SLACK) != hipSuccess ||
        (h->useTags && hipMalloc((void **) &h->tags, nSlots * sizeof(uint16_t)) != hipSuccess) ||
        hipMalloc((void **) &h->ht, (size_t) h->hash_size * sizeof(ht_entry)) != hipSuccess ||
        hipMalloc((void **) &h->lut, 256) != hipSuccess) {
        swsem_destroy(h);
        return fail(SWSEM_ENOMEM, "cannot allocate %llu B reference + %llu B hash table in HBM",
                    (unsigned long long) maxRefLength, (unsigned long long) h->hash_size * 8ull);
    }
    uint8_t lut[256];
    build_lut(lut);
    HIPCHK(hipMemcpy(h->lut, lut, 256, hipMemcpyHostToDevice));
    HIPCHK(hipMemsetAsync(h->ht, 0, (size_t) h->hash_size * sizeof(ht_entry), h->stream));
    if (h->tags) HIPCHK(hipMemsetAsync(h->tags, 0, nSlots * sizeof(uint16_t), h->stream));
    HIPCHK(hipMemsetAsync(h->ref, 0, maxRefLength, h->stream));
    HIPCHK(hipMemsetAsync(h->ref + maxRefLength, 0, REF_SLACK, h->stream));
    HIPCHK(hipStreamSynchronize(h->stream));
    *out = h;
    return SWSEM_OK;
}

void swsem_destroy(swsem_t *h) {
    if (!h) return;
    (void) hipSetDevice(h->device);
    for (auto &E : h->slot) E.deferred2b = false;
    for (hipStream_t s : {h->stream, h->stream2, h->stream3, h->streamUp, h->streamAux, h->streamLoad}) if (s) (void) hipStreamSynchronize(s);
    h->drain_events();
    if (h->sw.debugStats) {
        fprintf(stderr, "swsem stitch: blocks replayed %llu, accepted in runs %llu, tested one by one %llu, jumped over %llu\n",
                (unsigned long long) h->stitchDiag[0], (unsigned long long) h->stitchDiag[1], (unsigned long long) h->stitchDiag[2], (unsigned long long) h->stitchDiag[3]);
        uint64_t t[8];
        if (swsem_debug_emit_stats(h, t) == SWSEM_OK && (t[4] | t[5] | t[6] | t[7]))
            fprintf(stderr, "swsem pairing chain: foreign-boundary steps %llu, blocks not accepted %llu, groups replayed %llu, blocks given up %llu\n",
                    (unsigned long long) t[4], (unsigned long long) t[5], (unsigned long long) t[6], (unsigned long long) t[7]);
    }
    if (h->stream3) (void) hipStreamDestroy(h->stream3);
    if (h->ownStream && h->stream) (void) hipStreamDestroy(h->stream);
    delete h;
}

int swsem_set_stream(swsem_t *h, void *s) { MATCHER_ONLY(h);
    HIPCHK(hipStreamSynchronize(h->stream));
    if (h->ownStream) (void) hipStreamDestroy(h->stream);
    h->stream = (hipStream_t) s;
    h->ownStream = false;
    return deal_streams(h);
}
int swsem_synchronize(swsem_t *h) { HIPCHK(hipStreamSynchronize(h->stream)); return SWSEM_OK; }

void swsem_disable_sliding_window(swsem_t *h) { h->swSize = 0; h->ld.swEnd = h->circular ? 0 : h->maxRefLength; }
void swsem_set_sliding_window_size(swsem_t *h, int f) { h->swSize = h->maxRefLength / (uint64_t) (uint8_t) f; }
void swsem_disable_circular_buffer(swsem_t *h) { h->circular = false; h->ld.swEnd = h->maxRefLength; }
uint64_t swsem_get_ref_length(const swsem_t *h) { return h->refLength(); }
uint64_t swsem_get_loading_position(const swsem_t *h) { return (uint64_t) h->ld.pos1; }
uint64_t swsem_get_loaded_ref_length(const swsem_t *h) { return loaded_ref_length(h); }
uint64_t swsem_get_max_ref_length(const swsem_t *h) { return h->maxRefLength; }
uint64_t swsem_get_dropped_bytes(const swsem_t *h) { return h->ld.droppedBytes; }
uint64_t swsem_get_sliding_window_size(const swsem_t *h) { return h->circular ? h->swSize : 0; }
void swsem_set_position(swsem_t *h, uint64_t p, int laps) { h->ld.pos1 = (int64_t) p; h->ld.laps = laps; h->ld.pristine = false; }
int swsem_get_K(const swsem_t *h) { return h->K; }
uint32_t swsem_get_hash_size(const swsem_t *h) { return h->hash_size; }

uint64_t swsem_acquire_lock(swsem_t *h) {
    if (h->swSize == 0 || !h->circular) return h->ld.swEnd;
    uint64_t w = (uint64_t) h->ld.pos1 + h->swSize;
    if (h->ld.laps || w > h->maxRefLength) {
        if (w > h->maxRefLength) w -= h->maxRefLength - REF_SHIFT;
    } else
        w = h->maxRefLength;
    if (h->ld.locks.empty()) h->ld.swEnd = w;
    h->ld.locks.push_back(w);
    return w;
}

int swsem_release_lock(swsem_t *h, uint64_t v) { MATCHER_ONLY(h); return release_lock(h, v); }

int swsem_load_ref_dev(swsem_t *h, const uint8_t *t, uint64_t len, int loadRC, int addSep, int sep) { MATCHER_ONLY(h);
    HIPCHK(hipSetDevice(h->device));
    int r = load_pieces(h, t, len, false, addSep != 0, sep);
    if (r) return r;
    if (loadRC) r = load_pieces(h, t, len, true, addSep != 0, sep);
    return r;
}

int swsem_load_ref(swsem_t *h, const uint8_t *t, uint64_t len, int loadRC, int addSep, int sep) { MATCHER_ONLY(h);
    HIPCHK(hipSetDevice(h->device));
    if (len == 0) return SWSEM_OK;
    int r = h->stage.reserve(len + 64);
    if (r) return r;
    HIPCHK(hipMemcpyAsync(h->stage.p, t, len, hipMemcpyHostToDevice, h->stream));
    r = swsem_load_ref_dev(h, h->stage.p, len, loadRC, addSep, sep);
    if (r) return r;
    HIPCHK(hipStreamSynchronize(h->stream));
    return SWSEM_OK;
}
int swsem_load_separator(swsem_t *h, int sep) { MATCHER_ONLY(h);
    HIPCHK(hipSetDevice(h->device));
    return load_separator(h, sep);
}

int swsem_finalize_targets(swsem_t *h, int n, const uint8_t *const *ext_dev, const uint64_t *ext_len, int addSep, int sep,
                           int lazySeparator, const uint64_t *lockPos, uint64_t *loadedAfter) { MATCHER_ONLY(h);
    return finalize_impl(h, n, ext_dev, ext_len, addSep, sep, lazySeparator, lockPos, loadedAfter, nullptr);
}

int swsem_match_batch_dev(swsem_t *h, const uint8_t *q, const uint64_t *offsets, int n, uint32_t minLen, const uint64_t *lockPos) { MATCHER_ONLY(h);
    HIPCHK(hipSetDevice(h->device));
    return run_batch(h, q, offsets, n, minLen, lockPos);
}

int swsem_batch_counts(swsem_t *h, uint64_t *nm) { MATCHER_ONLY(h);
    if (!h->batchValid) return fail(SWSEM_EINVAL, "no batch results");
    if (h->matchCount.size() != h->contigs.size()) { int r = fetch_counts(h); if (r) return r; }
    for (size_t c = 0; c < h->contigs.size(); c++) nm[c] = h->matchCount[c];
    return SWSEM_OK;
}

int swsem_batch_matches(swsem_t *h, int c, swsem_match_t *out, uint64_t cap) { MATCHER_ONLY(h);
    if (!h->batchValid || c < 0 || c >= (int) h->contigs.size()) return fail(SWSEM_EINVAL, "no such contig in the batch");
    if (h->matchCount.size() != h->contigs.size()) { int r = fetch_counts(h); if (r) return r; }
    const uint64_t n = std::min<uint64_t>(cap, h->matchCount[c]);
    if (n) HIPCHK(hipMemcpy(out, h->dMatches.p + h->contigs[c].matchBase, n * sizeof(Match), hipMemcpyDeviceToHost));
    return SWSEM_OK;
}

int swsem_batch_fingerprint(swsem_t *h, uint64_t *fp, uint64_t *tot, uint64_t *len) { MATCHER_ONLY(h);
    if (!h->batchValid) return fail(SWSEM_EINVAL, "no batch results");
    k_fingerprint<<<1, 1, 0, h->stream>>>(h->dContigs.p, (int) h->contigs.size(), h->dMatches.p, h->dMatchCount.p, h->dStats.p + 4);
    unsigned long long o[3];
    HIPCHK(hipMemcpyAsync(o, h->dStats.p + 4, sizeof o, hipMemcpyDeviceToHost, h->stream));
    HIPCHK(hipStreamSynchronize(h->stream));
    *fp = o[0]; *tot = o[1]; *len = o[2];
    h->stats[3] = o[1]; h->stats[4] = o[2];
    return SWSEM_OK;
}

int swsem_match(swsem_t *h, const uint8_t *query, uint64_t len, uint32_t minLen, uint64_t lockPos,
                const swsem_match_t **matches, uint64_t *nmatches) { MATCHER_ONLY(h);
    HIPCHK(hipSetDevice(h->device));
    *matches = nullptr; *nmatches = 0;
    int r = swsem_emit_batch_end(h);
    if (r) return r;
    if ((r = h->stage.reserve(len + 64))) return r;
    if (len) HIPCHK(hipMemcpyAsync(h->stage.p, query, len, hipMemcpyHostToDevice, h->stream));
    const uint64_t offs[2] = {0, len};
    if ((r = run_batch(h, h->stage.p, offs, 1, minLen, &lockPos))) return r;
    if ((r = fetch_counts(h))) return r;
    h->hostMatches.resize(h->matchCount[0]);
    if (h->matchCount[0])
        HIPCHK(hipMemcpy(h->hostMatches.data(), h->dMatches.p, h->matchCount[0] * sizeof(Match), hipMemcpyDeviceToHost));
    *matches = h->hostMatches.data();
    *nmatches = h->matchCount[0];
    return SWSEM_OK;
}

int swsem_dev_malloc(swsem_t *h, uint64_t bytes, void **out) {
    HIPCHK(hipSetDevice(h->device));
    *out = nullptr;
    if (hipMalloc(out, bytes ? bytes : 1) != hipSuccess) return fail(SWSEM_ENOMEM, "device allocation of %llu bytes failed", (unsigned long long) bytes);
    return SWSEM_OK;
}
int swsem_dev_free(swsem_t *h, void *p) {
    HIPCHK(hipSetDevice(h->device));
    HIPCHK(hipStreamSynchronize(h->stream));
    if (p) HIPCHK(hipFree(p));
    return SWSEM_OK;
}
int swsem_dev_upload(swsem_t *h, void *dst_dev, const void *src, uint64_t bytes) {
    HIPCHK(hipSetDevice(h->device));
    if (bytes) HIPCHK(hipMemcpyAsync(dst_dev, src, bytes, hipMemcpyHostToDevice, h->stream));
    HIPCHK(hipStreamSynchronize(h->stream));
    return SWSEM_OK;
}
int swsem_dev_download(swsem_t *h, void *dst, const void *src_dev, uint64_t bytes) {
    HIPCHK(hipSetDevice(h->device));
    if (bytes) HIPCHK(hipMemcpyAsync(dst, src_dev, bytes, hipMemcpyDeviceToHost, h->stream));
    HIPCHK(hipStreamSynchronize(h->stream));
    return SWSEM_OK;
}
int swsem_dev_copy(swsem_t *h, void *dst_dev, const void *src_dev, uint64_t bytes) {
    HIPCHK(hipSetDevice(h->device));
    if (bytes) HIPCHK(hipMemcpyAsync(dst_dev, src_dev, bytes, hipMemcpyDeviceToDevice, h->stream));
    return SWSEM_OK;
}

int swsem_revcomp_dev(swsem_t *h, const uint8_t *src_dev, uint64_t n, uint8_t *dst_dev) {
    HIPCHK(hipSetDevice(h->device));
    if (n == 0) return SWSEM_OK;
    const uint64_t thr = (n + 3) / 4;
    const unsigned blocks = (unsigned) std::min<uint64_t>((thr + 255) / 256, 8192);
    h->mark(SWSEM_K_LOAD, true);
    k_load_rc<<<dim3(blocks), dim3(256), 0, h->stream>>>(src_dev, dst_dev, n, h->lut);
    h->mark(SWSEM_K_LOAD, false);
    HIPCHK(hipGetLastError());
    return SWSEM_OK;
}

int swsem_debug_copy_ref(swsem_t *h, uint64_t from, uint64_t n, uint8_t *out) {
    HIPCHK(hipStreamSynchronize(h->stream));
    HIPCHK(hipMemcpy(out, h->ref + from, n, hipMemcpyDeviceToHost));
    return SWSEM_OK;
}

int swsem_debug_write_ref(swsem_t *h, uint64_t from, uint64_t n, const uint8_t *in) { MATCHER_ONLY(h);
    if (from + n > h->maxRefLength) return fail(SWSEM_EINVAL, "swsem_debug_write_ref: beyond the buffer");
    HIPCHK(hipStreamSynchronize(h->stream));
    HIPCHK(hipStreamSynchronize(h->stream2));
    HIPCHK(hipMemcpy(h->ref + from, in, n, hipMemcpyHostToDevice));
    {
        const uint64_t s0 = from >= (uint64_t) h->K ? (from - h->K + 1) >> h->k1ord : 0, s1 = (from + n + ((1ull << h->k1ord) - 1)) >> h->k1ord;
        if (h->tags && s1 > s0) HIPCHK(hipMemset(h->tags + s0, 0, (s1 - s0) * sizeof(uint16_t)));
    }
    return SWSEM_OK;
}

int swsem_debug_copy_ht(swsem_t *h, uint32_t *out) { MATCHER_ONLY(h);
    DevBuf<uint32_t> tmp;
    int r = tmp.reserve(h->hash_size);
    if (r) return r;
    k_ht_low_words<<<dim3((h->hash_size + 255) / 256), dim3(256), 0, h->stream>>>(h->ht, tmp.p, h->hash_size, h->fpBits);
    HIPCHK(hipStreamSynchronize(h->stream));
    HIPCHK(hipMemcpy(out, tmp.p, (size_t) h->hash_size * 4, hipMemcpyDeviceToHost));
    return SWSEM_OK;
}

int swsem_debug_block_times(swsem_t *h, uint64_t *out, uint64_t cap, uint64_t *n) { MATCHER_ONLY(h);
    uint64_t nb = 0;
    for (auto &c : h->contigs) nb += c.nrb;
    *n = nb;
    if (nb > cap) nb = cap;
    std::vector<BlockRec> tmp(nb);
    HIPCHK(hipStreamSynchronize(h->stream));
    if (nb) HIPCHK(hipMemcpy(tmp.data(), h->dRecs.p, nb * sizeof(BlockRec), hipMemcpyDeviceToHost));
    for (uint64_t i = 0; i < nb; i++) { out[3 * i] = tmp[i].cycles; out[3 * i + 1] = tmp[i].visits; out[3 * i + 2] = tmp[i].emits; }
    return SWSEM_OK;
}

int swsem_debug_emit_stats(swsem_t *h, uint64_t out[8]) { MATCHER_ONLY(h);
    HIPCHK(hipDeviceSynchronize());
    for (int k = 0; k < 8; k++) out[k] = 0;
    for (auto &E : h->slot) {
        if (!E.dEStat.p || !E.statZeroed) continue;
        unsigned long long t[8];
        HIPCHK(hipMemcpy(t, E.dEStat.p, sizeof t, hipMemcpyDeviceToHost));
        for (int k = 0; k < 8; k++) out[k] += t[k];
    }
    return SWSEM_OK;
}

#ifdef SWSEM_DIAG_PHASES
int swsem_debug_phases(swsem_t *h, uint64_t *out) {
    HIPCHK(hipStreamSynchronize(h->stream));
    unsigned long long z[8] = {0};
    HIPCHK(hipMemcpyFromSymbol(out, HIP_SYMBOL(swk::g_diag), sizeof z));
    HIPCHK(hipMemcpyToSymbol(HIP_SYMBOL(swk::g_diag), z, sizeof z));
    return SWSEM_OK;
}
#endif

int swsem_profile_enable(swsem_t *h, int on) {
    h->drain_events();
    h->prof = on != 0;
    memset(h->profMs, 0, sizeof h->profMs);
    memset(h->profN, 0, sizeof h->profN);
    return SWSEM_OK;
}

int swsem_profile_get(swsem_t *h, double ms[SWSEM_K_COUNT], uint64_t n[SWSEM_K_COUNT]) {
    h->drain_events();
    for (int i = 0; i < SWSEM_K_COUNT; i++) { ms[i] = h->profMs[i]; n[i] = h->profN[i]; }
    return SWSEM_OK;
}

int swsem_batch_stats(swsem_t *h, uint64_t s[6]) { MATCHER_ONLY(h);
    if (!h->batchValid) return fail(SWSEM_EINVAL, "no batch results");
    for (int i = 0; i < 6; i++) s[i] = h->stats[i];
    return SWSEM_OK;
}

void swsem_emit_params_default(swsem_emit_params_t *p, int mode) {
    memset(p, 0, sizeof(*p));
    p->enableExtensionsWithMismatches = 1;
    p->mismatchesWithExclusion = 1;
    p->lazyDecompressionSupport = 1;
    p->enable40bitReference = 0;
    p->frugal64bitLenEncoding = 1;
    p->gapDepthOffsetEncoding = 64;
    p->gapDepthMismatchesEncoding = 2;
    p->gapBreakingMatchMinLength = 256;
    p->mmsMatchBonus = 50;
    p->mmsMismatchPenalty = 50;
    p->mmsMismatchesScoreThreshold = 500;
    p->mmsMismatchesInitialScore = 125;
    p->allowedTargetsOutrunForDissimilarContigs = 1;
    p->minimalLengthForDissimilarContigs = 1024;
    p->unmatchedFractionFactorTweakForDissimilarContigs = 16;
    if (mode == 0) {
        p->allowedTargetsOutrunForDissimilarContigs = 4;
        p->unmatchedFractionFactorTweakForDissimilarContigs = 32;
        p->frugal64bitLenEncoding = 0;
    }
    if (mode == 2) {
        p->allowedTargetsOutrunForDissimilarContigs = 0;
        p->unmatchedFractionFactorTweakForDissimilarContigs = 2;
    }
}

int swsem_emit_batch_begin(swsem_t *h, const swsem_emit_params_t *p, int n, const int *contigIdx, const uint64_t *lockPos,
                           const int *factor, const int64_t *processed, const int64_t *targetIdx,
                           const uint64_t *refExtLoadedPos, uint64_t nLoaded) { MATCHER_ONLY(h);
    return emit_begin_impl(h, p, n, contigIdx, lockPos, factor, processed, targetIdx, refExtLoadedPos, nLoaded, nullptr, nullptr);
}

int swsem_emit_batch_begin_spec(swsem_t *h, const swsem_emit_params_t *p, int n, const int *contigIdx, const uint64_t *lockPos,
                                const int *factor, const int64_t *processed, const int64_t *targetIdx,
                                const uint64_t *refExtLoadedPos, uint64_t nLoaded, const swsem_spec_finalize_t *spec, int *applied) { MATCHER_ONLY(h);
    return emit_begin_impl(h, p, n, contigIdx, lockPos, factor, processed, targetIdx, refExtLoadedPos, nLoaded, spec, applied);
}

int swsem_emit_batch_end(swsem_t *h) { MATCHER_ONLY(h);
    int r = end_slot(h, h->latest ^ 1);
    return r ? r : end_slot(h, h->latest);
}

int swsem_emit_select(swsem_t *h, int previous) { MATCHER_ONLY(h);
    h->selected = previous ? (h->latest ^ 1) : -1;
    return SWSEM_OK;
}

int swsem_emit_batch(swsem_t *h, const swsem_emit_params_t *p, int n, const int *contigIdx, const uint64_t *lockPos,
                     const int *factor, const int64_t *processed, const int64_t *targetIdx,
                     const uint64_t *refExtLoadedPos, uint64_t nLoaded) { MATCHER_ONLY(h);
    int r = swsem_emit_batch_begin(h, p, n, contigIdx, lockPos, factor, processed, targetIdx, refExtLoadedPos, nLoaded);
    return r ? r : swsem_emit_batch_end(h);
}

void swsem_emit_set_host_copy(swsem_t *h, int on) { h->emitHostCopy = on != 0; }

int swsem_emit_unmatched(swsem_t *h, uint64_t *unmatched) { MATCHER_ONLY(h);
    EmitSlot &E = h->slot[h->latest];
    for (size_t k = 0; k < E.eout.size(); k++) unmatched[k] = E.eout[k].unmatchedChars;
    return SWSEM_OK;
}

int swsem_emit_pack_dev(swsem_t *h, uint8_t *dst_dev, uint64_t cap, uint64_t *sizes, uint64_t *total) { MATCHER_ONLY(h);
    HIPCHK(hipSetDevice(h->device));
    EmitSlot &E = h->sel();
    { int e = end_slot(h, (int) (&E - h->slot)); if (e) return e; }
    if (sizes)
        for (size_t k = 0; k < E.eout.size(); k++)
            for (int st = 0; st < SWSEM_NSTREAMS; st++) sizes[k * SWSEM_NSTREAMS + st] = E.eout[k].size[st];
    if (dst_dev && E.packedBytes) {
        if (E.packedBytes > cap) return fail(SWSEM_EINVAL, "swsem_emit_pack_dev: buffer too small");
        HIPCHK(hipMemcpyAsync(dst_dev, E.dEArena.p, E.packedBytes, hipMemcpyDeviceToDevice, h->s3()));
        HIPCHK(hipStreamSynchronize(h->s3()));
    }
    if (total) *total = E.packedBytes;
    return SWSEM_OK;
}

int swsem_emit_pack_dev_on(swsem_t *h, uint8_t *dst_dev, uint64_t cap, void *stream) { MATCHER_ONLY(h);
    HIPCHK(hipSetDevice(h->device));
    EmitSlot &E = h->sel();
    { int e = end_slot(h, (int) (&E - h->slot)); if (e) return e; }
    if (!E.packedBytes) return SWSEM_OK;
    if (!dst_dev || E.packedBytes > cap) return fail(SWSEM_EINVAL, "swsem_emit_pack_dev_on: buffer too small");
    HIPCHK(hipMemcpyAsync(dst_dev, E.dEArena.p, E.packedBytes, hipMemcpyDeviceToDevice, stream ? (hipStream_t) stream : h->stream));
    return SWSEM_OK;
}

int swsem_emit_counters(swsem_t *h, uint64_t *out) { MATCHER_ONLY(h);
    EmitSlot &E = h->sel();
    { int e = end_slot(h, (int) (&E - h->slot)); if (e) return e; }
    for (size_t k = 0; k < E.eout.size(); k++) {
        const EmitOut &o = E.eout[k];
        const uint64_t v[6] = {o.unmatchedChars, o.extMatched, o.extMismatches, o.totalMatched, o.removed, o.nmatches};
        memcpy(out + k * 6, v, sizeof v);
    }
    return SWSEM_OK;
}

int swsem_emit_result(swsem_t *h, int k, swsem_streams_t *out) { MATCHER_ONLY(h);
    EmitSlot &E = h->sel();
    { int e = end_slot(h, (int) (&E - h->slot)); if (e) return e; }
    if (k < 0 || k >= (int) E.eout.size()) return fail(SWSEM_EINVAL, "swsem_emit_result: no result %d", k);
    if (!E.hostStreamsValid) {
        { int r = E.next_host_streams(E.packedBytes + 1); if (r) return r; }
        if (E.packedBytes) HIPCHK(hipMemcpyAsync(E.hostStreams().p, E.dEArena.p, E.packedBytes, hipMemcpyDeviceToHost, h->s3()));
        HIPCHK(hipStreamSynchronize(h->s3()));
        E.hostStreamsValid = true;
    }
    const EmitOut &o = E.eout[k];
    for (int st = 0; st < SWSEM_NSTREAMS; st++) {
        out->data[st] = E.hostStreams().p + E.hostStreamOff[(size_t) k * SWSEM_NSTREAMS + st];
        out->size[st] = o.size[st];
    }
    out->unmatchedChars = o.unmatchedChars;
    out->extensionsMatchedChars = o.extMatched;
    out->extensionsMismatches = o.extMismatches;
    out->totalMatched = o.totalMatched;
    out->removedGapBreakingMatches = o.removed;
    out->nmatches = o.nmatches;
    return SWSEM_OK;
}

int swsem_decode_contigs_dev(swsem_t *h, const swsem_emit_params_t *p, int n, const swsem_decode_job_t *jobs, uint64_t *destLen, int64_t *unmatched) {
    HIPCHK(hipSetDevice(h->device));
    if (n <= 0) return SWSEM_OK;
    std::vector<DecodeJob> jb(n);
    for (int k = 0; k < n; k++) {
        for (int st = 0; st < SWSEM_NSTREAMS; st++) { jb[k].stream[st] = jobs[k].stream_dev[st]; jb[k].size[st] = jobs[k].size[st]; }
        jb[k].refLockPos = jobs[k].refLockPos; jb[k].dest = jobs[k].dest_dev; jb[k].destCap = jobs[k].destCap; jb[k].expect = nullptr;
    }
    std::vector<DecodeOut> outs;
    int r = decode_jobs(h, p, n, jb, outs);
    if (r) return r;
    for (int k = 0; k < n; k++) { destLen[k] = outs[k].destLen; unmatched[k] = outs[k].unmatched; }
    return SWSEM_OK;
}

int swsem_create_decoder(swsem_t **out, uint64_t maxRefLength, int device) {
    *out = nullptr;
    if (maxRefLength < 64) return fail(SWSEM_EINVAL, "reference length limit %llu out of range", (unsigned long long) maxRefLength);
    int ndev = 0;
    if (hipGetDeviceCount(&ndev) != hipSuccess || ndev <= 0 || device >= ndev)
        return fail(SWSEM_ENODEV, "no HIP device %d (the HIP path has no CPU fallback)", device);
    HIPCHK(hipSetDevice(device));
    g_eventsFailed = false;
    swsem *h = new swsem();
    h->device = device;
    h->decoder = true;
    if (g_eventsFailed) { swsem_destroy(h); return fail(SWSEM_EHIP, "hipEventCreate failed"); }
    h->maxRefLength = maxRefLength;
    if (hipStreamCreateWithFlags(&h->stream, hipStreamNonBlocking) != hipSuccess) { swsem_destroy(h); return fail(SWSEM_EHIP, "hipStreamCreate failed"); }
    h->ownStream = true;
    if (hipMalloc((void **) &h->ref, maxRefLength + REF_SLACK) != hipSuccess || hipMalloc((void **) &h->lut, 256) != hipSuccess) {
        swsem_destroy(h);
        return fail(SWSEM_ENOMEM, "cannot allocate %llu B reference in HBM", (unsigned long long) maxRefLength);
    }
    uint8_t lut[256];
    build_lut(lut);
    HIPCHK(hipMemcpy(h->lut, lut, 256, hipMemcpyHostToDevice));
    HIPCHK(hipMemsetAsync(h->ref, 0, maxRefLength + REF_SLACK, h->stream));
    HIPCHK(hipStreamSynchronize(h->stream));
    *out = h;
    return SWSEM_OK;
}

int swsem_decode_plan_chain_dev(swsem_t *h, const swsem_emit_params_t *p, const uint8_t *const stream_dev[SWSEM_NSTREAMS], const uint64_t size[SWSEM_NSTREAMS],
                                int nstarts, const swsem_chain_start_t *starts, int ntargets, const uint32_t *seqCount, const uint64_t *lockPos,
                                uint64_t ncontigs, swsem_chain_contig_t *out, int *firstBadChain) {
    HIPCHK(hipSetDevice(h->device));
    if (nstarts <= 0 || ntargets <= 0 || !firstBadChain) return fail(SWSEM_EINVAL, "swsem_decode_plan_chain_dev: no chain start");
    ChainStreams S;
    for (int st = 0; st < SWSEM_NSTREAMS; st++) { S.p[st] = stream_dev[st]; S.n[st] = size[st]; }
    return decode_plan_chain(h, p, S, nstarts, starts, ntargets, seqCount, lockPos, ncontigs, out, firstBadChain);
}

int swsem_decode_fill_range_dev(swsem_t *h, uint64_t c0, uint64_t c1, uint8_t *dest_dev, const uint64_t *destOff, uint64_t *nbad) {
    HIPCHK(hipSetDevice(h->device));
    int r = decode_fill_range(h, c0, c1, dest_dev, destOff);
    if (r || !nbad) return r;
    std::vector<uint32_t> bad(c1 - c0);
    if (c1 > c0) HIPCHK(hipMemcpyAsync(bad.data(), h->chain.dBad.p + c0, (c1 - c0) * sizeof(uint32_t), hipMemcpyDeviceToHost, h->stream));
    HIPCHK(hipStreamSynchronize(h->stream));
    *nbad = 0;
    for (uint32_t b : bad) *nbad += b != 0;
    return SWSEM_OK;
}

int swsem_decode_load_dev(swsem_t *h, const uint8_t *src_dev, int n, const swsem_load_seg_t *segs) {
    HIPCHK(hipSetDevice(h->device));
    return decode_load(h, src_dev, n, segs);
}

int swsem_emit_verify(swsem_t *h, int *nbad, int *firstBad, uint64_t *firstDiff) {
    MATCHER_ONLY(h);
    HIPCHK(hipSetDevice(h->device));
    EmitSlot &E = h->sel();
    { int e = end_slot(h, (int) (&E - h->slot)); if (e) return e; }
    const int n = (int) E.eout.size();
    *nbad = 0; if (firstBad) *firstBad = -1; if (firstDiff) *firstDiff = UINT64_MAX;
    if (n == 0) return SWSEM_OK;
    uint64_t total = 0;
    for (int k = 0; k < n; k++) total += E.ecg[k].n + 16;
    int r;
    if ((r = h->dDecode.reserve(total))) return r;
    std::vector<DecodeJob> jb;
    std::vector<int> which;
    uint64_t at = 0;
    for (int k = 0; k < n; k++) {
        if (E.eout[k].unmatchedChars == UINT64_MAX) { at += E.ecg[k].n + 16; continue; }
        DecodeJob j;
        for (int st = 0; st < SWSEM_NSTREAMS; st++) { j.stream[st] = E.dEArena.p + E.hostStreamOff[(size_t) k * SWSEM_NSTREAMS + st]; j.size[st] = E.eout[k].size[st]; }
        j.refLockPos = E.ecg[k].lock; j.dest = h->dDecode.p + at; j.destCap = E.ecg[k].n; j.expect = E.qdev + E.ecg[k].qoff;
        at += E.ecg[k].n + 16;
        jb.push_back(j); which.push_back(k);
    }
    if (jb.empty()) return SWSEM_OK;
    std::vector<DecodeOut> outs;
    if ((r = decode_jobs(h, &E.params, (int) jb.size(), jb, outs))) return r;
    for (size_t i = 0; i < jb.size(); i++) {
        const int k = which[i];
        const bool ok = outs[i].unmatched >= 0 && outs[i].destLen == E.ecg[k].n && outs[i].firstDiff == UINT64_MAX &&
                        (uint32_t) outs[i].unmatched == (uint32_t) E.eout[k].unmatchedChars;
        if (!ok) {
            if (*nbad == 0) { if (firstBad) *firstBad = k; if (firstDiff) *firstDiff = outs[i].unmatched < 0 ? outs[i].destLen : outs[i].firstDiff; }
            (*nbad)++;
        }
    }
    return SWSEM_OK;
}

int swsem_emit(swsem_t *h, const swsem_emit_params_t *p, int contig, uint64_t lockPos, int factor, int64_t processed,
               int64_t targetIdx, const uint64_t *loaded, uint64_t nLoaded, swsem_streams_t *out) { MATCHER_ONLY(h);
    int r = swsem_emit_batch(h, p, 1, &contig, &lockPos, &factor, &processed, &targetIdx, loaded, nLoaded);
    if (r) return r;
    return swsem_emit_result(h, 0, out);
}

}
```

mbgc_amd/csrc/swsem_runtime_match.h:

```cpp
namespace {

bool build_resolve_order(swsem *h, uint32_t rblocks, uint32_t per) {
    std::vector<uint32_t> key;
    key.reserve(h->contigs.size() + 3);
    key.push_back(rblocks); key.push_back(per);
    for (auto &cg : h->contigs) key.push_back(cg.nrb);
    if (key == h->rbOrderKey && !h->rbOrderHost.empty()) return false;
    h->rbOrderKey.swap(key);
    std::vector<uint32_t> &order = h->rbOrderHost;
    order.clear();
    uint32_t maxNrb = 0;
    for (auto &cg : h->contigs) maxNrb = std::max(maxNrb, cg.nrb);
    std::vector<uint32_t> byLen(h->contigs.size());
    for (uint32_t c = 0; c < byLen.size(); c++) byLen[c] = c;
    std::stable_sort(byLen.begin(), byLen.end(), [&](uint32_t a, uint32_t b) { return h->contigs[a].nrb > h->contigs[b].nrb; });
    std::vector<uint32_t> lists[8];
    std::vector<uint32_t> grp;
    size_t alive = byLen.size();
    const size_t piece = 64;
    for (uint32_t b = 0; b < maxNrb; b++) {
        while (alive && h->contigs[byLen[alive - 1]].nrb <= b) alive--;
        grp.assign(byLen.begin(), byLen.begin() + alive);
        if (!std::is_sorted(grp.begin(), grp.end())) std::sort(grp.begin(), grp.end());
        for (size_t i = 0; i < grp.size(); i += piece) {
            int best = 0;
            for (int x = 1; x < 8; x++) if (lists[x].size() < lists[best].size()) best = x;
            const size_t e = std::min(grp.size(), i + piece);
            for (size_t k = i; k < e; k++) lists[best].push_back(h->contigs[grp[k]].rb0 + b);
            while (lists[best].size() % per) lists[best].push_back(0xFFFFFFFFu);
        }
    }
    size_t len = 0;
    for (auto &l : lists) len = std::max(len, l.size() / per);
    order.assign(len * 8 * per, 0xFFFFFFFFu);
    for (int x = 0; x < 8; x++)
        for (size_t j = 0; j < lists[x].size() / per; j++)
            for (uint32_t k = 0; k < per; k++) order[(j * 8 + x) * per + k] = lists[x][j * per + k];
    return true;
}

struct BatchShape {
    uint64_t matchRows = 0, bases = 0, probes = 0;
    uint32_t rblocks = 0;
    uint32_t rslots = 0;
    uint32_t cap = 0;
    bool blocks = false;
};

int batch_layout(swsem *h, const uint64_t *offsets, int n, uint32_t minLen, const uint64_t *lockPos, BatchShape &B) {
    h->contigs.assign(n, Contig());
    std::vector<uint32_t> &rbContig = h->rbContigHost;
    rbContig.clear();
    uint64_t allUnits = 0;
    for (int c = 0; c < n; c++) {
        const uint64_t len = offsets[c + 1] - offsets[c];
        allUnits += len >= (uint64_t) h->K ? (len - h->K + 1 + RBU - 1) / RBU : 0;
    }
    h->chainsPerWave = (h->sw.simt && !h->sw.seqResolve && h->K <= K_MAX4) ? (uint32_t) GC : 1u;
    const uint64_t waves = h->chainsPerWave > 1 ? (uint64_t) h->waveSlots / RESOLVE_WAVES_PER_SIMD * RESOLVE4_WAVES_PER_SIMD : h->waveSlots;
    const uint64_t slots = std::max<uint64_t>(1, waves * h->chainsPerWave * h->slotPercent / 100);
    h->rb = h->sw.rbFixed ? h->sw.rbFixed : (uint32_t) std::min<uint64_t>(65536 / RBU, std::max<uint64_t>(RB_MIN, (allUnits + slots - 1) / slots));
    for (int c = 0; c < n; c++) {
        Contig &cg = h->contigs[c];
        cg.qoff = offsets[c];
        cg.n = offsets[c + 1] - offsets[c];
        if (cg.n >= (1ull << 31) - (1ull << 20)) return fail(SWSEM_EINVAL, "contig %d longer than 2^31 - 2^20 bytes", c);
        cg.lock = lockPos ? lockPos[c] : UINT64_MAX;
        const uint64_t npos = cg.n >= (uint64_t) h->K ? cg.n - h->K + 1 : 0;
        B.probes += npos;
        cg.matchBase = B.matchRows;
        B.matchRows += cg.n / minLen + 2;
        cg.rb0 = B.rblocks;
        cg.nrb = (uint32_t) ((npos + (uint64_t) h->rb * RBU - 1) / ((uint64_t) h->rb * RBU));
        for (uint32_t t = 0; t < cg.nrb; t++) rbContig.push_back((uint32_t) c);
        B.rblocks += cg.nrb;
        B.bases += cg.n;
    }
    B.blocks = !h->sw.seqResolve && B.rblocks != 0;
    B.cap = (uint32_t) ((h->rb * RBU + OVERLAP_MAX + h->K) / h->K + 8);
    return SWSEM_OK;
}

int batch_upload(swsem *h, int n, BatchShape &B) {
    const uint32_t rblocks = B.rblocks;
    int r;
    if ((r = h->dContigs.reserve(n)) || (r = h->dMatchCount.reserve(n)) || (r = h->dStats.reserve(8)) || (r = h->dMatches.reserve(B.matchRows))) return r;
    if (B.blocks && ((r = h->dRegions.reserve((size_t) rblocks * B.cap)) || (r = h->dReplay.reserve((size_t) n * B.cap)) || (r = h->dRecs.reserve(rblocks)) ||
                     (r = h->dFast.reserve(rblocks)) || (r = h->dSegStart.reserve(rblocks)) || (r = h->dKeepN.reserve(rblocks)) ||
                     (r = h->dDstOff.reserve(rblocks)) || (r = h->dPrev.reserve(rblocks))))
        return r;
    if ((r = upload(h, h->dContigs.p, h->contigs.data(), n * sizeof(Contig), h->stream))) return r;
    if ((r = h->dRbContig.reserve(std::max<uint32_t>(rblocks, 1)))) return r;
    if (rblocks) {
        const uint32_t *had = h->dRbOrder.p;
        const bool fresh = build_resolve_order(h, rblocks, h->chainsPerWave);
        B.rslots = (uint32_t) (h->rbOrderHost.size() / h->chainsPerWave);
        if ((r = h->dRbOrder.reserve(h->rbOrderHost.size() + h->rbOrderHost.size() / 4 + 64))) return r;
        if ((r = upload(h, h->dRbContig.p, h->rbContigHost.data(), rblocks * sizeof(uint32_t), h->stream))) return r;
        if ((fresh || had != h->dRbOrder.p) && (r = upload(h, h->dRbOrder.p, h->rbOrderHost.data(), h->rbOrderHost.size() * sizeof(uint32_t), h->stream)))
            return r;
    }
    if ((r = zero_dev(h, h->dStats.p, 8 * sizeof(unsigned long long), h->stream))) return r;
    return flush_copies(h);
}

int batch_launch(swsem *h, const uint8_t *qdev, int n, const BatchShape &B) {
    const uint32_t rblocks = B.rblocks, rslots = B.rslots, cap = B.cap;
    int r;
    const RefView v = h->view();
    const bool wrapped = v.fpCheck == 2;
    if (!B.blocks)
        for (auto &E : h->slot) if ((r = run_phase2b(h, E, false))) return r;
    HIPCHK(hipEventRecord(h->evRoundTop, h->stream));
    h->roundTopFresh = true;
    if (!B.blocks) {
        h->mark(SWSEM_K_RESOLVE, true);
        if (wrapped) k_resolve_seq<true><<<dim3(n), dim3(WAVE), 0, h->stream>>>(v, qdev, h->dContigs.p, h->dMatches.p, h->dMatchCount.p);
        else k_resolve_seq<false><<<dim3(n), dim3(WAVE), 0, h->stream>>>(v, qdev, h->dContigs.p, h->dMatches.p, h->dMatchCount.p);
        h->mark(SWSEM_K_RESOLVE, false);
    } else {
        h->batchBlocks = rblocks;
        if (h->metaPending) { HIPCHK(hipStreamWaitEvent(h->stream, h->evMeta, 0)); h->metaPending = false; }
        bool anyDeferred = false;
        for (auto &E : h->slot) anyDeferred |= E.deferred2b;
        if (anyDeferred) HIPCHK(hipEventRecord(h->evFin, h->stream));
        h->mark(SWSEM_K_RESOLVE, true);
        if (h->chainsPerWave == (uint32_t) GC) {
            if (wrapped) k_resolve_blocks4<true><<<dim3(rslots), dim3(WAVE), 0, h->stream>>>(v, qdev, h->dContigs.p, h->dRbContig.p, h->dRbOrder.p, h->dRegions.p, cap, h->rb, h->dRecs.p, h->overlap);
            else k_resolve_blocks4<false><<<dim3(rslots), dim3(WAVE), 0, h->stream>>>(v, qdev, h->dContigs.p, h->dRbContig.p, h->dRbOrder.p, h->dRegions.p, cap, h->rb, h->dRecs.p, h->overlap);
        } else {
            if (wrapped) k_resolve_blocks<true><<<dim3(rslots), dim3(WAVE), 0, h->stream>>>(v, qdev, h->dContigs.p, h->dRbContig.p, h->dRbOrder.p, h->dRegions.p, cap, h->rb, h->dRecs.p, h->overlap);
            else k_resolve_blocks<false><<<dim3(rslots), dim3(WAVE), 0, h->stream>>>(v, qdev, h->dContigs.p, h->dRbContig.p, h->dRbOrder.p, h->dRegions.p, cap, h->rb, h->dRecs.p, h->overlap);
        }
        h->mark(SWSEM_K_RESOLVE, false);
        if (anyDeferred) {
            HIPCHK(hipStreamWaitEvent(h->stream2, h->evFin, 0));
            for (auto &E : h->slot) if ((r = run_phase2b(h, E, true))) return r;
        }
        h->mark(SWSEM_K_STITCH, true);
        k_stitch_pre<<<dim3((rblocks + 255) / 256), dim3(256), 0, h->stream>>>(h->dContigs.p, h->dRbContig.p, h->dRecs.p, h->rb, rblocks, h->dFast.p);
        if (wrapped) k_stitch<true><<<dim3(n), dim3(WAVE), 0, h->stream>>>(v, qdev, h->dContigs.p, h->dRegions.p, h->dReplay.p, cap, h->rb, h->dRecs.p, h->dFast.p, h->dSegStart.p,
                                                                          h->dKeepN.p, h->dPrev.p, h->dDstOff.p, h->dMatchCount.p, h->dStats.p);
        else k_stitch<false><<<dim3(n), dim3(WAVE), 0, h->stream>>>(v, qdev, h->dContigs.p, h->dRegions.p, h->dReplay.p, cap, h->rb, h->dRecs.p, h->dFast.p, h->dSegStart.p,
                                                                    h->dKeepN.p, h->dPrev.p, h->dDstOff.p, h->dMatchCount.p, h->dStats.p);
        k_gather<<<dim3(rblocks), dim3(WAVE), 0, h->stream>>>(h->dContigs.p, h->dRbContig.p, h->dRegions.p, cap, h->dSegStart.p,
                                                            h->dKeepN.p, h->dDstOff.p, h->dMatches.p);
        h->mark(SWSEM_K_STITCH, false);
    }
    HIPCHK(hipGetLastError());
    HIPCHK(hipEventRecord(h->evMatched, h->stream));
    return SWSEM_OK;
}

int run_batch(swsem *h, const uint8_t *qdev, const uint64_t *offsets, int n, uint32_t minLen, const uint64_t *lockPos) {
    if (n <= 0) return fail(SWSEM_EINVAL, "empty batch");
    if (minLen < (uint32_t) h->K)
        return fail(SWSEM_EINVAL, "Minimal matching length cannot be smaller than K (%u < %d)", minLen, h->K);
    h->batchValid = false;
    h->matchCount.clear();
    h->minLen = minLen;
    BatchShape B;
    int r;
    if ((r = batch_layout(h, offsets, n, minLen, lockPos, B)) || (r = batch_upload(h, n, B)) || (r = batch_launch(h, qdev, n, B))) return r;
    h->qdev = qdev;
    h->stats[0] = B.bases;
    h->hostProbes = B.probes;
    h->batchValid = true;
    return SWSEM_OK;
}

int queue_counts(swsem *h, size_t extraBytes, hipStream_t st = nullptr) {
    if (!st) st = h->stream;
    const size_t n = h->contigs.size();
    const size_t countsAt = 64, extraAt = (countsAt + n * sizeof(uint32_t) + 63) & ~(size_t) 63;
    const size_t bytes = extraAt + extraBytes;
    int r = h->pin.reserve(bytes, std::max<size_t>(2 * bytes, 1 << 20));
    if (r) return r;
    if ((r = download(h, h->pin.p, h->dStats.p, 8 * sizeof(unsigned long long), st)) ||
        (r = download(h, h->pin.p + countsAt, h->dMatchCount.p, n * sizeof(uint32_t), st)))
        return r;
    h->pinExtraAt = extraAt;
    return SWSEM_OK;
}

void take_counts(swsem *h) {
    const size_t n = h->contigs.size();
    const unsigned long long *st = (const unsigned long long *) h->pin.p;
    h->matchCount.assign((const uint32_t *) (h->pin.p + 64), (const uint32_t *) (h->pin.p + 64) + n);
    h->stats[1] = h->hostProbes; h->stats[2] = st[2]; h->stats[5] = st[3];
    h->stitchDiag[0] += st[3]; h->stitchDiag[1] += st[5]; h->stitchDiag[2] += st[6]; h->stitchDiag[3] += st[7];
    if (h->batchBlocks >= 2048) {
        const uint64_t replayed = st[3];
        if (replayed * 400 > h->batchBlocks) h->overlap = std::min<uint32_t>((uint32_t) OVERLAP_MAX, h->overlap + 128);
        else if (replayed * 2000 < h->batchBlocks) h->overlap = std::max<uint32_t>(640u, h->overlap - 128);
        h->batchBlocks = 0;
    }
    uint64_t tot = 0;
    for (size_t c = 0; c < n; c++) tot += h->matchCount[c];
    h->stats[3] = tot;
}

int fetch_counts(swsem *h) {
    int r = queue_counts(h, 0);
    if (r || (r = flush_copies(h))) return r;
    HIPCHK(hipStreamSynchronize(h->stream));
    take_counts(h);
    return SWSEM_OK;
}

}
```

mbgc_amd/csrc/swsem_runtime_state.h:

```cpp
#define SWSEM_ESPEC (-100)

namespace {

thread_local std::string g_err;
int fail(int code, const char *fmt, ...) {
    char buf[512];
    va_list ap;
    va_start(ap, fmt);
    vsnprintf(buf, sizeof buf, fmt, ap);
    va_end(ap);
    g_err = buf;
    return code;
}
#define HIPCHK(x) do { hipError_t e_ = (x); if (e_ != hipSuccess) return fail(SWSEM_EHIP, "%s: %s", #x, hipGetErrorString(e_)); } while (0)

constexpr uint64_t REF_SHIFT = 1;
constexpr int SW_WIDTH_FACTOR = 16;
constexpr uint64_t REF_SLACK = 256;
constexpr uint64_t COPY_WGS = 2048;
constexpr uint32_t EMIT_THIN_MAX = 512;
constexpr uint32_t RB_MIN = 2048 / RBU;

struct NoCopy {
    NoCopy() = default;
    NoCopy(const NoCopy &) = delete;
    NoCopy &operator=(const NoCopy &) = delete;
};
template <typename T>
struct DevBuf : NoCopy {
    T *p = nullptr;
    size_t cap = 0;
    ~DevBuf() { if (p) (void) hipFree(p); }
    int reserve(size_t n) {
        if (n <= cap) return SWSEM_OK;
        if (p) (void) hipFree(p);
        p = nullptr; cap = 0;
        size_t want = n + n / 8 + 64;
        if (hipMalloc((void **) &p, want * sizeof(T)) != hipSuccess) {
            p = nullptr;
            return fail(SWSEM_ENOMEM, "device allocation of %zu bytes failed", want * sizeof(T));
        }
        cap = want;
        return SWSEM_OK;
    }
};

struct PinBuf : NoCopy {
    uint8_t *p = nullptr;
    size_t cap = 0;
    ~PinBuf() { if (p) (void) hipHostFree(p); }
    int reserve(size_t bytes, size_t want, unsigned flags = hipHostMallocCoherent | hipHostMallocMapped) {
        if (bytes <= cap) return SWSEM_OK;
        if (p) (void) hipHostFree(p);
        p = nullptr; cap = 0;
        if (hipHostMalloc((void **) &p, want, flags) != hipSuccess) {
            p = nullptr;
            return fail(SWSEM_ENOMEM, "cannot pin %zu B of host memory", want);
        }
        cap = want;
        return SWSEM_OK;
    }
};

thread_local bool g_eventsFailed = false;
struct Event : NoCopy {
    hipEvent_t e = nullptr;
    Event() { if (hipEventCreateWithFlags(&e, hipEventDisableTiming) != hipSuccess) { e = nullptr; g_eventsFailed = true; } }
    ~Event() { if (e) (void) hipEventDestroy(e); }
    operator hipEvent_t() const { return e; }
};

struct ProfEvent { hipEvent_t a, b; int fam; };

struct LoaderState {
    int64_t pos1 = REF_SHIFT;
    int laps = 0;
    uint64_t samplingPos = 0, swEnd = 0;
    std::deque<uint64_t> locks;
    uint32_t epoch = 1;
    uint32_t eCur = 0, ePrev = 0;
    int64_t sepEndPos = -1; int sepEndLaps = -1, sepEndVal = -1;
    bool pristine = true;
    uint64_t droppedBytes = 0;

    bool sep_end_done(int sep) const { return pos1 == sepEndPos && laps == sepEndLaps && sep == sepEndVal; }
    void sep_end_set(int64_t at, int sep) { sepEndPos = at; sepEndLaps = laps; sepEndVal = sep; }
    uint64_t refLength(uint64_t maxRefLength) const { return laps ? maxRefLength : (uint64_t) pos1; }
    void wrap_if_at_end(uint64_t maxRefLength) {
        if ((uint64_t) pos1 != maxRefLength || swEnd == maxRefLength) return;
        laps++;
        ePrev = eCur; eCur = epoch;
        pos1 = REF_SHIFT;
        samplingPos = REF_SHIFT;
    }
};

struct Switches {
    bool seqResolve = false;
    bool simt = true;
    uint32_t rbFixed = 0;
    uint32_t profMask = ~0u;
    int metaWarm = swk::MWARM;
    bool lapTags = true;
    bool streamCalib = true;
    bool streamDebug = false;
    bool debugStats = false;
};
Switches read_switches() {
    Switches s;
    if (const char *e = getenv("SWSEM_RESOLVE")) s.seqResolve = strcmp(e, "seq") == 0;
    if (const char *e = getenv("SWSEM_CHAINS")) s.simt = atoi(e) != 1;
    if (const char *e = getenv("SWSEM_RB")) { int x = atoi(e); if (x >= 1 && x <= 256) s.rbFixed = (uint32_t) x * (1024 / RBU); }
    if (const char *e = getenv("SWSEM_PROF_FAMS")) s.profMask = (uint32_t) strtoul(e, nullptr, 0);
    if (const char *e = getenv("SWSEM_META_WARM")) s.metaWarm = std::min(swk::MWARM, std::max(0, atoi(e)));
    if (const char *e = getenv("SWSEM_LAP_TAGS")) s.lapTags = atoi(e) != 0;
    if (const char *e = getenv("SWSEM_STREAM_CALIB")) s.streamCalib = atoi(e) != 0;
    s.streamDebug = getenv("SWSEM_STREAM_DEBUG") != nullptr;
    s.debugStats = getenv("SWSEM_DEBUG_STATS") != nullptr;
    return s;
}

struct PreparedInserts {
    size_t np = 0, nc = 0, nb = 0, ne = 0;
    bool beside = false;
    uint64_t nSamples = 0, nEdge = 0, copyBlocks = 0;
    const InsertPiece *dPieces = nullptr, *dEdge = nullptr;
    const uint64_t *dFirst = nullptr, *dCFirst = nullptr, *dEFirst = nullptr;
    const CopyPiece *dCopies = nullptr;
    const BytePiece *dBytes = nullptr;
};

struct EmitSlot {
    DevBuf<EmitContig> dECg;
    DevBuf<EmitOut> dEOut;
    DevBuf<int> dEWhich;
    DevBuf<uint32_t> dEOwner, dESpanOwner;
    DevBuf<EMatch> dEM;
    DevBuf<uint64_t> dENext0, dELoaded, dEPack;
    DevBuf<uint8_t> dERm, dEArena;
    DevBuf<uint32_t> dEKeep, dEMeta, dECorr, dESz, dEOfs, dEChunk;
    DevBuf<MetaRec> dEStates;
    DevBuf<unsigned long long> dEStat, dEPm, dELit, dEBad;
    DevBuf<LongCopy> dELong;
    DevBuf<uint32_t> dELongCount;
    bool statZeroed = false;
    std::vector<EmitContig> ecg;
    std::vector<uint32_t> chunkOwner, spanOwner;
    std::vector<int> ewhich;
    std::vector<uint64_t> eloaded;
    std::vector<EmitOut> eout;
    Event evDone;
    Event evMetaDone;
    bool outstanding = false, refGuarded = false;
    bool donePending = false;
    bool deferred2b = false, waitFin2b = false;
    EmitView v2b; uint32_t grid2b = 0; int n2b = 0;
    const uint8_t *qdev = nullptr;
    swsem_emit_params_t params;
    uint64_t emitPos1 = 0;
    uint64_t lockMin = UINT64_MAX;
    int emitLaps = 0;
    int emitN = 0;
    PinBuf pinE;
    PinBuf hostHalf[2];
    int hostAt = 0;
    PinBuf &hostStreams() { return hostHalf[hostAt]; }
    int next_host_streams(size_t n) { hostAt ^= 1; return hostStreams().reserve(n, n + n / 2 + 4096, hipHostMallocDefault); }
    std::vector<uint64_t> hostStreamOff;
    bool hostStreamsValid = false;
    uint64_t packedBytes = 0;
};

}

struct swsem {
    int device = 0;
    hipStream_t stream = nullptr;
    bool ownStream = false;
    Switches sw;
    uint8_t *ref = nullptr;
    ht_entry *ht = nullptr;
    uint8_t *lut = nullptr;
    uint16_t *tags = nullptr;
    bool useTags = true;
    LoaderState ld;
    uint64_t maxRefLength = 0;
    int L = 0, K = 0, k1 = 0, skipMargin = 0, k1ord = 0;
    uint32_t hash_size = 0, mask = 0;
    uint64_t swSize = 0;
    bool circular = true;
    int fpBits = 0;
    uint64_t hostProbes = 0;
    bool deferInserts = false;
    bool specMode = false;
    DevBuf<uint32_t> dGate;
    DevBuf<uint8_t> dPred;
    std::vector<InsertPiece> pendingPieces;
    std::vector<InsertPiece> edgePieces;
    int prioLow = 0, prioHigh = 0;
    Event evLoadFork, evLoadDone;
    std::vector<CopyPiece> pendingCopies;
    std::vector<BytePiece> pendingBytes;
    DevBuf<uint64_t> dTables;
    struct HostTab { PinBuf buf; Event ev; bool pending = false; } hostTables[2];
    int hostTableSel = 0;
    PreparedInserts prep;
    hipStream_t stream2 = nullptr, streamLoad = nullptr, streamUp = nullptr, streamAux = nullptr;
    Event evTables, evRoundTop;
    bool roundTopFresh = false;
    DevBuf<uint8_t> stage;
    DevBuf<Contig> dContigs;
    DevBuf<uint32_t> dMatchCount, dRbContig, dRbOrder;
    std::vector<uint32_t> rbOrderHost, rbOrderKey;
    uint32_t chainsPerWave = 1;
    hipStream_t stream3 = nullptr;
    hipStream_t s3() {
        if (!stream3 && hipStreamCreateWithFlags(&stream3, hipStreamNonBlocking) != hipSuccess) stream3 = stream;
        return stream3;
    }
    Event evMatched;
    std::vector<uint32_t> rbContigHost;
    DevBuf<Match> dMatches;
    DevBuf<Row> dRegions, dReplay;
    DevBuf<BlockRec> dRecs;
    DevBuf<FastRec> dFast;
    DevBuf<uint32_t> dSegStart, dKeepN, dDstOff;
    DevBuf<int32_t> dPrev;
    DevBuf<unsigned long long> dStats;
    DevBuf<uint8_t> dDecode;
    DevBuf<DecodeJob> dJobs;
    DevBuf<DecRec> dDecRecs;
    DevBuf<DecPlanOut> dDecPlan;
    DevBuf<uint64_t> dDecAux;
    bool decoder = false;
    struct ChainState {
        DevBuf<ChainStart> dStarts;
        DevBuf<ChainContig> dContigs;
        DevBuf<uint32_t> dSeqCount, dChainBad, dBad;
        DevBuf<uint64_t> dLock, dRecBase;
        DevBuf<LoadSeg> dSegs;
        ChainStreams streams = {};
        swsem_emit_params_t params = {};
        uint64_t n = 0;
        std::vector<uint64_t> nrec, destLen, litEnd, lock;
        const uint8_t *jobsDest = nullptr;
    } chain;
    EmitSlot slot[2];
    int latest = 0;
    uint64_t capN = 0, capRows = 0, capArena = 0, capLoaded = 0, capChunks = 0;
    int selected = -1;
    EmitSlot &sel() { return slot[selected < 0 ? latest : selected]; }
    PinBuf pin; size_t pinExtraAt = 0;
    PinBuf ring; size_t ringAt = 0;
    Event evP1;
    Event evFin;
    Event evMeta;
    bool metaPending = false;
    bool emitHostCopy = true;
    uint32_t overlap = 1024, batchBlocks = 0;
    uint32_t rb = 8;
    uint64_t stitchDiag[4] = {0, 0, 0, 0};
    uint32_t slotPercent = 95;
    uint32_t waveSlots = 256 * 4 * RESOLVE_WAVES_PER_SIMD;
    std::vector<Contig> contigs;
    std::vector<uint32_t> matchCount;
    std::vector<swsem_match_t> hostMatches;
    const uint8_t *qdev = nullptr;
    uint32_t minLen = 0;
    bool batchValid = false;
    uint64_t stats[6] = {0, 0, 0, 0, 0, 0};
    bool prof = false;
    std::deque<ProfEvent> events;
    double profMs[SWSEM_K_COUNT] = {0};
    uint64_t profN[SWSEM_K_COUNT] = {0};

    CopySegs segs;
    hipStream_t segStream = nullptr;

    uint64_t refLength() const { return ld.refLength(maxRefLength); }
    RefView view() const {
        RefView v;
        v.ref = ref; v.ht = ht; v.pos1 = (uint64_t) ld.pos1; v.refLength = refLength(); v.maxRefLength = maxRefLength;
        v.mask = mask; v.fpBits = fpBits; v.fpCheck = (fpBits && ld.pristine) ? (ld.laps ? 2 : 1) : 0; v.eCur = ld.eCur; v.ePrev = ld.ePrev;
        v.curMax = ld.pos1 >= (int64_t) K + 1 ? (uint32_t) (((uint64_t) ld.pos1 - K - 1) >> k1ord) : 0u;
        v.prevMin = (uint32_t) ((((uint64_t) ld.pos1) + (1ull << k1ord) - 1) >> k1ord); v.K = K; v.k1ord = k1ord; v.skipMargin = skipMargin; v.minLen = minLen;
        v.tags = useTags ? tags : nullptr; v.tagCur = swk::lap_tag(ld.laps); v.tagPrev = ld.laps ? swk::lap_tag(ld.laps - 1) : 0u;
        return v;
    }
    std::vector<ProfEvent> idle;
    void account(const ProfEvent &e) {
        float ms = 0;
        (void) hipEventElapsedTime(&ms, e.a, e.b);
        profMs[e.fam] += ms; profN[e.fam]++;
        idle.push_back(e);
    }
    void mark(int fam, bool begin, hipStream_t on = nullptr) {
        if (!prof || !((sw.profMask >> fam) & 1u)) return;
        if (!on) on = stream;
        if (begin) {
            while (events.size() > 1 && hipEventQuery(events.front().b) == hipSuccess) {
                account(events.front());
                events.pop_front();
            }
            ProfEvent e;
            if (!idle.empty()) { e = idle.back(); idle.pop_back(); }
            else { (void) hipEventCreate(&e.a); (void) hipEventCreate(&e.b); }
            e.fam = fam;
            (void) hipEventRecord(e.a, on);
            events.push_back(e);
        } else
            (void) hipEventRecord(events.back().b, on);
    }
    void drain_events() {
        for (auto &e : events) {
            (void) hipEventSynchronize(e.b);
            account(e);
        }
        events.clear();
    }
    ~swsem() {
        for (void *p : {(void *) ref, (void *) tags, (void *) ht, (void *) lut}) if (p) (void) hipFree(p);
        drain_events();
        for (auto &e : idle) { (void) hipEventDestroy(e.a); (void) hipEventDestroy(e.b); }
    }
};
```

Measured before the change: 52.18.

## Precompute stitch replays for candidate blocks in parallel before sequential stitch

Adds a k_stitch_replay kernel that, for blocks whose boundary with the previous block is decidable but mismatched, speculatively replays the chain in parallel (one wave per candidate) and stores the resulting rows. The sequential per-contig k_stitch can then take these precomputed replays instead of running chain_run serially, which shortens the serial critical path. It also retunes the adaptive overlap thresholds (lower floor, more sensitive to replay rate) and adds an env override. The cost is an extra kernel launch, scratch memory (up to 4096 candidates), and wasted work when candidates are refused.

```diff
diff --git a/include/mbgc_swsem.h b/include/mbgc_swsem.h
--- a/include/mbgc_swsem.h
+++ b/include/mbgc_swsem.h
@@ -169,7 +169,7 @@
 int swsem_debug_block_times(swsem_t *h, uint64_t *out , uint64_t cap, uint64_t *nblocks);
 int swsem_profile_enable(swsem_t *h, int on);
 int swsem_profile_get(swsem_t *h, double ms[SWSEM_K_COUNT], uint64_t launches[SWSEM_K_COUNT]);
-int swsem_batch_stats(swsem_t *h, uint64_t stats[6]);
+int swsem_batch_stats(swsem_t *h, uint64_t stats[9]);
 
 #ifdef __cplusplus
 }
diff --git a/mbgc_amd/binding.py b/mbgc_amd/binding.py
--- a/mbgc_amd/binding.py
+++ b/mbgc_amd/binding.py
@@ -263,9 +263,10 @@
         return fp.value, tot.value, ln.value
 
     def batch_stats(self):
-        s = (C.c_uint64 * 6)()
+        s = (C.c_uint64 * 9)()
         _chk(lib().swsem_batch_stats(self.h, s))
-        return dict(zip(("bases", "probes", "hits", "matches", "matched_len", "replayed_blocks"), s))
+        return dict(zip(("bases", "probes", "hits", "matches", "matched_len", "replayed_blocks", "replays_precomputed",
+                         "candidates_unused", "candidates_refused"), s))
 
     def emit(self, params, contig=0, lock=NO_LOCK, factor=128, processed=0, target_idx=0, loaded=None):
         ld = np.ascontiguousarray(loaded if loaded is not None else [0], dtype=np.uint64)
diff --git a/mbgc_amd/csrc/swsem_kernels.hip b/mbgc_amd/csrc/swsem_kernels.hip
--- a/mbgc_amd/csrc/swsem_kernels.hip
+++ b/mbgc_amd/csrc/swsem_kernels.hip
@@ -678,9 +678,11 @@
     int32_t npush;
     int32_t popB;
 };
+constexpr uint32_t NO_CAND = 0xFFFFFFFFu;
 __global__ void __launch_bounds__(256) k_stitch_pre(const Contig *__restrict__ contigs, const uint32_t *__restrict__ rbContig,
                                                     const BlockRec *__restrict__ recs, uint32_t rb, uint32_t nblocks,
-                                                    FastRec *__restrict__ fast) {
+                                                    FastRec *__restrict__ fast, uint32_t *__restrict__ candOf,
+                                                    uint32_t *__restrict__ candBlock, unsigned long long *__restrict__ candCount, uint32_t bound) {
     const uint32_t g = blockIdx.x * blockDim.x + threadIdx.x;
     if (g >= nblocks) return;
     const Contig cg = contigs[rbContig[g]];
@@ -689,6 +691,7 @@
     FastRec f;
     f.scanF = (int32_t) cur.scanF; f.minKeep = cur.minKeep; f.npush = cur.spF - cur.minKeep; f.popB = -1;
     const bool visited = cur.minTouched != 0x7fffffff;
+    uint32_t slot = NO_CAND;
     if (b == 0) {
         if (visited) f.popB = 0;
     } else if (visited && cur.minTouched >= 0) {
@@ -697,13 +700,149 @@
         const int32_t pScanF = (int32_t) prv.scanF;
         const int cmp = cur.spB - cur.minTouched;
         const int prevPush = prv.spF - prv.minKeep;
-        bool ok = prv.minTouched != 0x7fffffff && pScanF < w0 + span && (pScanF > w0 ? pScanF : w0) == (int32_t) cur.scanB &&
-                  cmp >= 0 && cmp <= SNAP && cmp <= prevPush;
+        const bool decidable = prv.minTouched != 0x7fffffff && pScanF < w0 + span && cmp >= 0 && cmp <= SNAP && cmp <= prevPush;
+        bool ok = decidable && (pScanF > w0 ? pScanF : w0) == (int32_t) cur.scanB;
         for (int j = 0; ok && j < cmp; j++)
             ok = cur.bTop[j].posSrc == prv.fTop[j].posSrc && cur.bTop[j].len == prv.fTop[j].len && cur.bTop[j].posDest == prv.fTop[j].posDest;
         if (ok) f.popB = cur.spB - cur.minKeep;
+        else if (decidable) {
+            const unsigned long long s = atomicAdd(candCount, 1ull);
+            if (s < (unsigned long long) bound) { slot = (uint32_t) s; candBlock[slot] = g; }
+        }
     }
     fast[g] = f;
+    candOf[g] = slot;
+}
+
+struct __attribute__((aligned(16))) CandRec {
+    int32_t scan0;
+    int32_t scanEnd;
+    int32_t n;
+    int32_t removed;
+    int32_t examined;
+    int32_t usable;
+    int32_t specFrom, specN;
+};
+
+struct SeedStack : ArrayStack<Row> {
+    uint64_t lastSrc, lastLen, lastDest;
+    __device__ __forceinline__ void truncate_push(int keep, const Match &m, int32_t scanAfter) {
+        lastSrc = m.posSrc; lastLen = m.len; lastDest = m.posDest;
+        ArrayStack<Row>::truncate_push(keep, m, scanAfter);
+    }
+};
+constexpr int SPECW = 256;
+
+template <bool LAPS>
+__global__ void __launch_bounds__(WAVE) k_stitch_replay(RefView v, const uint8_t *__restrict__ qbuf,
+                                                        const Contig *__restrict__ contigs, const uint32_t *__restrict__ rbContig,
+                                                        Row *__restrict__ regions, Row *__restrict__ candArea,
+                                                        uint32_t cap, uint32_t rb, const BlockRec *__restrict__ recs,
+                                                        const uint32_t *__restrict__ candBlock, const unsigned long long *__restrict__ candCount,
+                                                        uint32_t bound, CandRec *__restrict__ cand,
+                                                        const uint32_t *__restrict__ candOf, FastRec *__restrict__ fast) {
+    __shared__ uint2 ring[RING];
+    __shared__ uint4 specA[SPECW];
+    __shared__ int32_t specB[SPECW];
+    const uint32_t slot = blockIdx.x;
+    if (slot >= bound || (unsigned long long) slot >= *candCount) return;
+    const uint32_t lane = threadIdx.x;
+    const uint32_t g = rfl32(candBlock[slot]);
+    const Contig cg = contigs[rbContig[g]];
+    const uint32_t b = g - cg.rb0;
+    const BlockRec *cur = recs + g, *prv = recs + g - 1;
+    const uint8_t *q = qbuf + cg.qoff;
+    const int32_t span = (int32_t) (rb * RBU), w0 = (int32_t) b * span;
+    const int32_t npos = cg.n >= (uint64_t) v.K ? (int32_t) (cg.n - v.K + 1) : 0;
+    const int32_t w1 = w0 + span < npos ? w0 + span : npos;
+    const int32_t room = (int32_t) cap + SNAP;
+    Row *scratch = candArea + (uint64_t) slot * (uint64_t) (room + (int32_t) cap);
+    Row *spec = regions + (uint64_t) g * cap;
+    const int spF = (int) rfl32((uint32_t) cur->spF), cMinKeep = (int) rfl32((uint32_t) cur->minKeep);
+    const int specFrom = cMinKeep < 0 ? 0 : cMinKeep;
+    const int specN = spF > specFrom ? spF - specFrom : 0;
+    for (int k = (int) lane; k < specN && k < SPECW; k += WAVE) {
+        const Row x = spec[specFrom + k];
+        specA[k] = make_uint4((uint32_t) x.posDest, (uint32_t) x.len, (uint32_t) x.posSrc, (uint32_t) (x.posSrc >> 32));
+        specB[k] = (int32_t) x.scanAfter;
+    }
+    SeedStack stk;
+    stk.st = scratch; stk.ring = ring; stk.sp = 0; stk.ringLow = 0; stk.lastSrc = stk.lastLen = stk.lastDest = 0;
+    const int32_t pSpF = (int32_t) rfl32((uint32_t) prv->spF);
+    const int nSeed = pSpF < SNAP ? pSpF : SNAP;
+    for (int j = 0; j < nSeed; j++) {
+        Match m;
+        m.posSrc = rfl64(prv->fTop[nSeed - 1 - j].posSrc); m.len = rfl64(prv->fTop[nSeed - 1 - j].len); m.posDest = rfl64(prv->fTop[nSeed - 1 - j].posDest);
+        stk.truncate_push(j, m, 0);
+    }
+    const int32_t pScanF = (int32_t) rfl32((uint32_t) prv->scanF);
+    Chain ch;
+    ch.scan = pScanF > w0 ? pScanF : w0; ch.minTouched = 0x7fffffff; ch.minKeep = 0x7fffffff; ch.visited = 0; ch.cands = 0; ch.emitted = false;
+    const int32_t scan0 = ch.scan;
+    int sp = specFrom;
+    int syncAt = -1;
+    bool full = false;
+    auto spec_row = [&](int at, uint32_t &pos, uint32_t &len, uint64_t &src, int32_t &scanAfter) {
+        if (at - specFrom < SPECW) {
+            const uint4 a = specA[at - specFrom];
+            pos = rfl32(a.x); len = rfl32(a.y); src = ((uint64_t) rfl32(a.w) << 32) | rfl32(a.z); scanAfter = (int32_t) rfl32((uint32_t) specB[at - specFrom]);
+        } else {
+            pos = rfl32((uint32_t) spec[at].posDest); len = rfl32((uint32_t) spec[at].len); src = rfl64(spec[at].posSrc); scanAfter = (int32_t) rfl32((uint32_t) spec[at].scanAfter);
+        }
+    };
+    auto stop = [&]() -> bool {
+        if (stk.sp >= room - 1) { full = true; return true; }
+        if (!ch.emitted) return false;
+        ch.emitted = false;
+        const uint32_t ePos = (uint32_t) stk.lastDest;
+        uint32_t pos = 0, len = 0; uint64_t src = 0; int32_t after = 0;
+        while (sp < spF) {
+            spec_row(sp, pos, len, src, after);
+            if (pos >= ePos) break;
+            sp++;
+        }
+        if (sp < spF && pos == ePos && len == (uint32_t) stk.lastLen && src == stk.lastSrc && after == ch.scan) { syncAt = sp; return true; }
+        return false;
+    };
+    chain_run<LAPS>(v, cg, q, w0, w1, stk, ch, stop);
+    __builtin_amdgcn_s_waitcnt(0);
+    CandRec r;
+    r.scan0 = scan0; r.specFrom = specFrom; r.specN = specN;
+    const int first = ch.minKeep < nSeed ? ch.minKeep : nSeed;
+    r.removed = nSeed - first;
+    r.examined = !ch.visited || ch.minTouched >= nSeed ? 0 : nSeed - ch.minTouched;
+    int n = stk.sp - first;
+    bool usable = !full && !(ch.visited && ch.minTouched < 0) && r.removed <= r.examined && n >= 0;
+    r.scanEnd = ch.scan;
+    if (usable && syncAt >= 0) {
+        const int tail = spF - syncAt - 1;
+        if (stk.sp + tail > room) usable = false;
+        else {
+            for (int k = (int) lane; k < tail; k += WAVE) scratch[stk.sp + k] = spec[syncAt + 1 + k];
+            n += tail;
+            r.scanEnd = (int32_t) rfl32((uint32_t) cur->scanF);
+        }
+    }
+    if (n > (int) cap || specN > (int) cap) usable = false;
+    r.n = n; r.usable = usable ? 1 : 0;
+    if (lane == 0) cand[slot] = r;
+    if (!usable) return;
+    Row *saved = scratch + room;
+    for (int k = (int) lane; k < specN; k += WAVE) saved[k] = spec[specFrom + k];
+    __builtin_amdgcn_s_waitcnt(0);
+    for (int k = (int) lane; k < n; k += WAVE) spec[k] = scratch[first + k];
+    const int prevPush = pSpF - (int) rfl32((uint32_t) prv->minKeep);
+    if (rfl32(candOf[g - 1]) != NO_CAND || r.examined > prevPush) return;
+    if (lane == 0) {
+        FastRec f;
+        f.scanF = r.scanEnd; f.minKeep = 0; f.npush = n; f.popB = r.removed;
+        fast[g] = f;
+    }
+    if (b + 1 < cg.nrb && rfl32(candOf[g + 1]) == NO_CAND && (int32_t) rfl32((uint32_t) fast[g + 1].popB) >= 0) {
+        const BlockRec *nxt = recs + g + 1;
+        const int cmpNext = (int) rfl32((uint32_t) nxt->spB) - (int) rfl32((uint32_t) nxt->minTouched);
+        if (!(syncAt >= 0 && cmpNext <= spF - syncAt) && lane == 0) fast[g + 1].popB = -1;
+    }
 }
 
 template <bool LAPS>
@@ -715,7 +854,9 @@
                                                  uint32_t *__restrict__ segStart, uint32_t *__restrict__ keepN,
                                                  int32_t *__restrict__ prev, uint32_t *__restrict__ dstOff,
                                                  uint32_t *__restrict__ matchCount,
-                                                 unsigned long long *__restrict__ stats) {
+                                                 unsigned long long *__restrict__ stats,
+                                                 const uint32_t *__restrict__ candOf, const CandRec *__restrict__ cand,
+                                                 const Row *__restrict__ candArea) {
     const Contig cg = contigs[blockIdx.x];
     const uint32_t lane = threadIdx.x;
     const uint8_t *q = qbuf + cg.qoff;
@@ -730,14 +871,28 @@
     __shared__ uint64_t ptop[TW];
     int known = 0;
     uint32_t replayed = 0, nFast = 0, nSlow = 0, nSkip = 0;
+    uint32_t nTaken = 0, nRefused = 0;
+    auto refresh_top = [&]() {
+        __builtin_amdgcn_s_waitcnt(0);
+        const int n = vs.size_ < SNAP ? vs.size_ : SNAP;
+        for (int j = 0; j < n; j++) {
+            const Row *m = vs.at(vs.size_ - 1 - j);
+            if (lane < 3) ptop[3 * j + lane] = ((const uint64_t *) m)[lane];
+        }
+        known = n;
+    };
     const BlockRec *rc = recs + cg.rb0;
     const int32_t span = (int32_t) (rb * RBU);
     const int32_t npos = cg.n >= (uint64_t) v.K ? (int32_t) (cg.n - v.K + 1) : 0;
     __shared__ uint4 srec[sizeof(BlockRec) / 16];
     bool prevPlain = true;
     uint4 fr = make_uint4(0, 0, 0, 0);
+    uint32_t cf = NO_CAND;
     for (uint32_t b = 0; b < cg.nrb; b++) {
-        if ((b & (WAVE - 1)) == 0) fr = b + lane < cg.nrb ? ((const uint4 *) (fast + cg.rb0))[b + lane] : make_uint4(0, 0, 0, 0xFFFFFFFFu);
+        if ((b & (WAVE - 1)) == 0) {
+            fr = b + lane < cg.nrb ? ((const uint4 *) (fast + cg.rb0))[b + lane] : make_uint4(0, 0, 0, 0xFFFFFFFFu);
+            cf = b + lane < cg.nrb ? candOf[cg.rb0 + b + lane] : NO_CAND;
+        }
         const int32_t w0 = (int32_t) b * span;
         if (scanT >= w0 + span) { prevPlain = false; nSkip++; continue; }
         const int fl = (int) (b & (WAVE - 1));
@@ -776,14 +931,20 @@
             known = 0;
             b += (uint32_t) (L - 1);
             nFast += (uint32_t) L;
+            const uint32_t nRep = (uint32_t) __popcll(__ballot(inRun && cf != NO_CAND));
+            replayed += nRep; nTaken += nRep;
             continue;
         }
         nSlow++;
+        const uint32_t ci = rl32(cf, fl);
         {
             const uint4 *src = (const uint4 *) (rc + b);
             for (uint32_t i = lane; i < sizeof(BlockRec) / 16; i += WAVE) srec[i] = src[i];
             __builtin_amdgcn_s_waitcnt(0);
         }
+        const CandRec *cr = cand + (ci == NO_CAND ? 0u : ci);
+        const bool swapped = ci != NO_CAND && rfl32((uint32_t) cr->usable) != 0;
+        const Row *saved = candArea + (uint64_t) (ci == NO_CAND ? 0u : ci) * (uint64_t) (2 * cap + SNAP) + (cap + SNAP);
         const BlockRec *r = (const BlockRec *) srec;
         const int32_t rScanB = (int32_t) rfl32((uint32_t) r->scanB), rScanF = (int32_t) rfl32((uint32_t) r->scanF);
         const int spB = (int) rfl32((uint32_t) r->spB), spF = (int) rfl32((uint32_t) r->spF);
@@ -798,15 +959,7 @@
                 const int cmp = minTouched < 0 ? spB : spB - minTouched;
                 if (minTouched < 0) ok = vs.size_ == spB && spB <= SNAP;
                 else ok = cmp <= SNAP && cmp <= vs.size_;
-                if (ok && cmp > known) {
-                    __builtin_amdgcn_s_waitcnt(0);
-                    const int n = vs.size_ < SNAP ? vs.size_ : SNAP;
-                    for (int j = 0; j < n; j++) {
-                        const Row *m = vs.at(vs.size_ - 1 - j);
-                        if (lane < 3) ptop[3 * j + lane] = ((const uint64_t *) m)[lane];
-                    }
-                    known = n;
-                }
+                if (ok && cmp > known) refresh_top();
                 if (ok) {
                     const bool diff = (int) lane < 3 * cmp && bw[lane < TW ? lane : 0] != ptop[lane < TW ? lane : 0];
                     ok = __ballot(diff) == 0;
@@ -814,6 +967,12 @@
             }
         }
         if (ok) {
+            if (swapped) {
+                const int sFrom = (int) rfl32((uint32_t) cr->specFrom), sN = (int) rfl32((uint32_t) cr->specN);
+                Row *dst = vs.region + (uint64_t) b * cap + sFrom;
+                for (int k = (int) lane; k < sN; k += WAVE) dst[k] = saved[k];
+                __builtin_amdgcn_s_waitcnt(0);
+            }
             if (visited || b == 0) {
                 const int popB = spB - minKeep;
                 const int npush = spF - minKeep;
@@ -833,12 +992,34 @@
                 prevPlain = true;
             } else
                 prevPlain = false;
+        } else if ([&]() -> bool {
+            if (ci == NO_CAND) return false;
+            const int32_t cScan0 = (int32_t) rfl32((uint32_t) cr->scan0), cExam = (int32_t) rfl32((uint32_t) cr->examined);
+            bool good = swapped && (scanT > w0 ? scanT : w0) == cScan0 && cExam <= vs.size_;
+            if (good && cExam > 0) {
+                if (cExam > known) refresh_top();
+                const uint64_t *pf = (const uint64_t *) rc[b - 1].fTop;
+                const bool diff = (int) lane < 3 * cExam && pf[lane < TW ? lane : 0] != ptop[lane < TW ? lane : 0];
+                good = __ballot(diff) == 0;
+            }
+            if (!good) { nRefused++; return false; }
+            const int32_t cRem = (int32_t) rfl32((uint32_t) cr->removed), cN = (int32_t) rfl32((uint32_t) cr->n);
+            if (cRem > 0) vs.pop_segments(cRem);
+            vs.size_ -= cRem;
+            vs.push_segment((int) b, 0, (uint32_t) cN);
+            scanT = (int32_t) rfl32((uint32_t) cr->scanEnd);
+            known = 0;
+            nTaken++;
+            return true;
+        }()) {
+            prevPlain = false;
+            replayed++;
         } else {
             prevPlain = false;
             Chain ch;
             ch.scan = scanT; ch.minTouched = 0x7fffffff; ch.minKeep = 0x7fffffff; ch.visited = 0; ch.cands = 0; ch.emitted = false;
             Row *own = replayArea + (uint64_t) blockIdx.x * cap;
-            const Row *spec = vs.region + (uint64_t) b * cap;
+            const Row *spec = swapped ? saved - (int) rfl32((uint32_t) cr->specFrom) : vs.region + (uint64_t) b * cap;
             vs.own = own; vs.ownN = 0;
             int sp = minKeep < 0 ? 0 : minKeep;
             int syncAt = -1;
@@ -893,6 +1074,8 @@
         atomicAdd(&stats[5], (unsigned long long) nFast);
         atomicAdd(&stats[6], (unsigned long long) nSlow);
         atomicAdd(&stats[7], (unsigned long long) nSkip);
+        if (nTaken) atomicAdd(&stats[9], (unsigned long long) nTaken);
+        if (nRefused) atomicAdd(&stats[10], (unsigned long long) nRefused);
     }
 }
 
diff --git a/mbgc_amd/csrc/swsem_runtime.hip b/mbgc_amd/csrc/swsem_runtime.hip
--- a/mbgc_amd/csrc/swsem_runtime.hip
+++ b/mbgc_amd/csrc/swsem_runtime.hip
@@ -103,6 +103,7 @@
     h->device = device;
     if (g_eventsFailed) { swsem_destroy(h); return fail(SWSEM_EHIP, "hipEventCreate failed"); }
     h->sw = read_switches();
+    if (h->sw.overlapFixed >= 0) h->overlap = (uint32_t) h->sw.overlapFixed;
     h->maxRefLength = maxRefLength;
     h->L = L; h->k1 = k1; h->skipMargin = skipMargin;
     h->k1ord = __builtin_ctz((unsigned) k1);
@@ -147,6 +148,8 @@
     if (h->sw.debugStats) {
         fprintf(stderr, "swsem stitch: blocks replayed %llu, accepted in runs %llu, tested one by one %llu, jumped over %llu\n",
                 (unsigned long long) h->stitchDiag[0], (unsigned long long) h->stitchDiag[1], (unsigned long long) h->stitchDiag[2], (unsigned long long) h->stitchDiag[3]);
+        fprintf(stderr, "swsem stitch: replayed ahead of the walk %llu, taken %llu, refused and replayed in place %llu, most in one batch %llu, warm-up positions at the end %u\n",
+                (unsigned long long) h->stitchDiag[4], (unsigned long long) h->stitchDiag[5], (unsigned long long) h->stitchDiag[6], (unsigned long long) h->stitchDiag[7], h->overlap);
         uint64_t t[8];
         if (swsem_debug_emit_stats(h, t) == SWSEM_OK && (t[4] | t[5] | t[6] | t[7]))
             fprintf(stderr, "swsem pairing chain: foreign-boundary steps %llu, blocks not accepted %llu, groups replayed %llu, blocks given up %llu\n",
@@ -390,9 +393,9 @@
     return SWSEM_OK;
 }
 
-int swsem_batch_stats(swsem_t *h, uint64_t s[6]) { MATCHER_ONLY(h);
+int swsem_batch_stats(swsem_t *h, uint64_t s[9]) { MATCHER_ONLY(h);
     if (!h->batchValid) return fail(SWSEM_EINVAL, "no batch results");
-    for (int i = 0; i < 6; i++) s[i] = h->stats[i];
+    for (int i = 0; i < 9; i++) s[i] = h->stats[i];
     return SWSEM_OK;
 }
 
diff --git a/mbgc_amd/csrc/swsem_runtime_match.h b/mbgc_amd/csrc/swsem_runtime_match.h
--- a/mbgc_amd/csrc/swsem_runtime_match.h
+++ b/mbgc_amd/csrc/swsem_runtime_match.h
@@ -45,6 +45,7 @@
     uint32_t rslots = 0;
     uint32_t cap = 0;
     bool blocks = false;
+    uint32_t cands = 0;
 };
 
 int batch_layout(swsem *h, const uint64_t *offsets, int n, uint32_t minLen, const uint64_t *lockPos, BatchShape &B) {
@@ -78,16 +79,18 @@
     }
     B.blocks = !h->sw.seqResolve && B.rblocks != 0;
     B.cap = (uint32_t) ((h->rb * RBU + OVERLAP_MAX + h->K) / h->K + 8);
+    B.cands = (uint32_t) std::min<uint64_t>(std::min<uint64_t>(B.rblocks, CAND_MAX), std::max<uint64_t>(1, CAND_BYTES / ((2 * B.cap + SNAP) * sizeof(Row))));
     return SWSEM_OK;
 }
 
 int batch_upload(swsem *h, int n, BatchShape &B) {
     const uint32_t rblocks = B.rblocks;
     int r;
-    if ((r = h->dContigs.reserve(n)) || (r = h->dMatchCount.reserve(n)) || (r = h->dStats.reserve(8)) || (r = h->dMatches.reserve(B.matchRows))) return r;
+    if ((r = h->dContigs.reserve(n)) || (r = h->dMatchCount.reserve(n)) || (r = h->dStats.reserve(NSTATS)) || (r = h->dMatches.reserve(B.matchRows))) return r;
     if (B.blocks && ((r = h->dRegions.reserve((size_t) rblocks * B.cap)) || (r = h->dReplay.reserve((size_t) n * B.cap)) || (r = h->dRecs.reserve(rblocks)) ||
                      (r = h->dFast.reserve(rblocks)) || (r = h->dSegStart.reserve(rblocks)) || (r = h->dKeepN.reserve(rblocks)) ||
-                     (r = h->dDstOff.reserve(rblocks)) || (r = h->dPrev.reserve(rblocks))))
+                     (r = h->dDstOff.reserve(rblocks)) || (r = h->dPrev.reserve(rblocks)) || (r = h->dCandOf.reserve(rblocks)) ||
+                     (r = h->dCandBlock.reserve(B.cands)) || (r = h->dCand.reserve(B.cands)) || (r = h->dCandArea.reserve((size_t) B.cands * (2 * B.cap + SNAP)))))
         return r;
     if ((r = upload(h, h->dContigs.p, h->contigs.data(), n * sizeof(Contig), h->stream))) return r;
     if ((r = h->dRbContig.reserve(std::max<uint32_t>(rblocks, 1)))) return r;
@@ -100,7 +103,7 @@
         if ((fresh || had != h->dRbOrder.p) && (r = upload(h, h->dRbOrder.p, h->rbOrderHost.data(), h->rbOrderHost.size() * sizeof(uint32_t), h->stream)))
             return r;
     }
-    if ((r = zero_dev(h, h->dStats.p, 8 * sizeof(unsigned long long), h->stream))) return r;
+    if ((r = zero_dev(h, h->dStats.p, NSTATS * sizeof(unsigned long long), h->stream))) return r;
     return flush_copies(h);
 }
 
@@ -119,7 +122,7 @@
         else k_resolve_seq<false><<<dim3(n), dim3(WAVE), 0, h->stream>>>(v, qdev, h->dContigs.p, h->dMatches.p, h->dMatchCount.p);
         h->mark(SWSEM_K_RESOLVE, false);
     } else {
-        h->batchBlocks = rblocks;
+        h->batchBlocks = rblocks; h->batchCands = B.cands;
         if (h->metaPending) { HIPCHK(hipStreamWaitEvent(h->stream, h->evMeta, 0)); h->metaPending = false; }
         bool anyDeferred = false;
         for (auto &E : h->slot) anyDeferred |= E.deferred2b;
@@ -138,11 +141,17 @@
             for (auto &E : h->slot) if ((r = run_phase2b(h, E, true))) return r;
         }
         h->mark(SWSEM_K_STITCH, true);
-        k_stitch_pre<<<dim3((rblocks + 255) / 256), dim3(256), 0, h->stream>>>(h->dContigs.p, h->dRbContig.p, h->dRecs.p, h->rb, rblocks, h->dFast.p);
+        unsigned long long *candCount = h->dStats.p + 8;
+        k_stitch_pre<<<dim3((rblocks + 255) / 256), dim3(256), 0, h->stream>>>(h->dContigs.p, h->dRbContig.p, h->dRecs.p, h->rb, rblocks, h->dFast.p,
+                                                                               h->dCandOf.p, h->dCandBlock.p, candCount, B.cands);
+        if (wrapped) k_stitch_replay<true><<<dim3(B.cands), dim3(WAVE), 0, h->stream>>>(v, qdev, h->dContigs.p, h->dRbContig.p, h->dRegions.p, h->dCandArea.p, cap, h->rb, h->dRecs.p,
+                                                                                       h->dCandBlock.p, candCount, B.cands, h->dCand.p, h->dCandOf.p, h->dFast.p);
+        else k_stitch_replay<false><<<dim3(B.cands), dim3(WAVE), 0, h->stream>>>(v, qdev, h->dContigs.p, h->dRbContig.p, h->dRegions.p, h->dCandArea.p, cap, h->rb, h->dRecs.p,
+                                                                                 h->dCandBlock.p, candCount, B.cands, h->dCand.p, h->dCandOf.p, h->dFast.p);
         if (wrapped) k_stitch<true><<<dim3(n), dim3(WAVE), 0, h->stream>>>(v, qdev, h->dContigs.p, h->dRegions.p, h->dReplay.p, cap, h->rb, h->dRecs.p, h->dFast.p, h->dSegStart.p,
-                                                                          h->dKeepN.p, h->dPrev.p, h->dDstOff.p, h->dMatchCount.p, h->dStats.p);
+                                                                          h->dKeepN.p, h->dPrev.p, h->dDstOff.p, h->dMatchCount.p, h->dStats.p, h->dCandOf.p, h->dCand.p, h->dCandArea.p);
         else k_stitch<false><<<dim3(n), dim3(WAVE), 0, h->stream>>>(v, qdev, h->dContigs.p, h->dRegions.p, h->dReplay.p, cap, h->rb, h->dRecs.p, h->dFast.p, h->dSegStart.p,
-                                                                    h->dKeepN.p, h->dPrev.p, h->dDstOff.p, h->dMatchCount.p, h->dStats.p);
+                                                                    h->dKeepN.p, h->dPrev.p, h->dDstOff.p, h->dMatchCount.p, h->dStats.p, h->dCandOf.p, h->dCand.p, h->dCandArea.p);
         k_gather<<<dim3(rblocks), dim3(WAVE), 0, h->stream>>>(h->dContigs.p, h->dRbContig.p, h->dRegions.p, cap, h->dSegStart.p,
                                                             h->dKeepN.p, h->dDstOff.p, h->dMatches.p);
         h->mark(SWSEM_K_STITCH, false);
@@ -172,11 +181,11 @@
 int queue_counts(swsem *h, size_t extraBytes, hipStream_t st = nullptr) {
     if (!st) st = h->stream;
     const size_t n = h->contigs.size();
-    const size_t countsAt = 64, extraAt = (countsAt + n * sizeof(uint32_t) + 63) & ~(size_t) 63;
+    const size_t countsAt = NSTATS * sizeof(unsigned long long), extraAt = (countsAt + n * sizeof(uint32_t) + 63) & ~(size_t) 63;
     const size_t bytes = extraAt + extraBytes;
     int r = h->pin.reserve(bytes, std::max<size_t>(2 * bytes, 1 << 20));
     if (r) return r;
-    if ((r = download(h, h->pin.p, h->dStats.p, 8 * sizeof(unsigned long long), st)) ||
+    if ((r = download(h, h->pin.p, h->dStats.p, NSTATS * sizeof(unsigned long long), st)) ||
         (r = download(h, h->pin.p + countsAt, h->dMatchCount.p, n * sizeof(uint32_t), st)))
         return r;
     h->pinExtraAt = extraAt;
@@ -186,13 +195,17 @@
 void take_counts(swsem *h) {
     const size_t n = h->contigs.size();
     const unsigned long long *st = (const unsigned long long *) h->pin.p;
-    h->matchCount.assign((const uint32_t *) (h->pin.p + 64), (const uint32_t *) (h->pin.p + 64) + n);
+    const uint32_t *counts = (const uint32_t *) (h->pin.p + NSTATS * sizeof(unsigned long long));
+    h->matchCount.assign(counts, counts + n);
+    const uint64_t cands = std::min<uint64_t>(st[8], h->batchCands);
     h->stats[1] = h->hostProbes; h->stats[2] = st[2]; h->stats[5] = st[3];
+    h->stats[6] = st[9]; h->stats[7] = cands - std::min<uint64_t>(cands, st[9]); h->stats[8] = st[10];
     h->stitchDiag[0] += st[3]; h->stitchDiag[1] += st[5]; h->stitchDiag[2] += st[6]; h->stitchDiag[3] += st[7];
-    if (h->batchBlocks >= 2048) {
+    h->stitchDiag[4] += cands; h->stitchDiag[5] += st[9]; h->stitchDiag[6] += st[10]; h->stitchDiag[7] = std::max<uint64_t>(h->stitchDiag[7], st[8]);
+    if (h->batchBlocks >= 2048 && h->sw.overlapFixed < 0) {
         const uint64_t replayed = st[3];
-        if (replayed * 400 > h->batchBlocks) h->overlap = std::min<uint32_t>((uint32_t) OVERLAP_MAX, h->overlap + 128);
-        else if (replayed * 2000 < h->batchBlocks) h->overlap = std::max<uint32_t>(640u, h->overlap - 128);
+        if (replayed * 40 > h->batchBlocks) h->overlap = std::min<uint32_t>((uint32_t) OVERLAP_MAX, h->overlap + 128);
+        else if (replayed * 160 < h->batchBlocks) h->overlap = std::max<uint32_t>(384u, h->overlap - 128);
         h->batchBlocks = 0;
     }
     uint64_t tot = 0;
diff --git a/mbgc_amd/csrc/swsem_runtime_state.h b/mbgc_amd/csrc/swsem_runtime_state.h
--- a/mbgc_amd/csrc/swsem_runtime_state.h
+++ b/mbgc_amd/csrc/swsem_runtime_state.h
@@ -20,6 +20,9 @@
 constexpr uint64_t COPY_WGS = 2048;
 constexpr uint32_t EMIT_THIN_MAX = 512;
 constexpr uint32_t RB_MIN = 2048 / RBU;
+constexpr uint32_t CAND_MAX = 4096;
+constexpr uint64_t CAND_BYTES = 128ull << 20;
+constexpr int NSTATS = 16;
 
 struct NoCopy {
     NoCopy() = default;
@@ -99,6 +102,7 @@
     bool seqResolve = false;
     bool simt = true;
     uint32_t rbFixed = 0;
+    int overlapFixed = -1;
     uint32_t profMask = ~0u;
     int metaWarm = swk::MWARM;
     bool lapTags = true;
@@ -111,6 +115,7 @@
     if (const char *e = getenv("SWSEM_RESOLVE")) s.seqResolve = strcmp(e, "seq") == 0;
     if (const char *e = getenv("SWSEM_CHAINS")) s.simt = atoi(e) != 1;
     if (const char *e = getenv("SWSEM_RB")) { int x = atoi(e); if (x >= 1 && x <= 256) s.rbFixed = (uint32_t) x * (1024 / RBU); }
+    if (const char *e = getenv("SWSEM_OVERLAP")) { int x = atoi(e); if (x >= 0 && x <= swk::OVERLAP_MAX) s.overlapFixed = x; }
     if (const char *e = getenv("SWSEM_PROF_FAMS")) s.profMask = (uint32_t) strtoul(e, nullptr, 0);
     if (const char *e = getenv("SWSEM_META_WARM")) s.metaWarm = std::min(swk::MWARM, std::max(0, atoi(e)));
     if (const char *e = getenv("SWSEM_LAP_TAGS")) s.lapTags = atoi(e) != 0;
@@ -224,6 +229,9 @@
     DevBuf<Row> dRegions, dReplay;
     DevBuf<BlockRec> dRecs;
     DevBuf<FastRec> dFast;
+    DevBuf<uint32_t> dCandOf, dCandBlock;
+    DevBuf<CandRec> dCand;
+    DevBuf<Row> dCandArea;
     DevBuf<uint32_t> dSegStart, dKeepN, dDstOff;
     DevBuf<int32_t> dPrev;
     DevBuf<unsigned long long> dStats;
@@ -257,9 +265,9 @@
     Event evMeta;
     bool metaPending = false;
     bool emitHostCopy = true;
-    uint32_t overlap = 1024, batchBlocks = 0;
+    uint32_t overlap = 1024, batchBlocks = 0, batchCands = 0;
     uint32_t rb = 8;
-    uint64_t stitchDiag[4] = {0, 0, 0, 0};
+    uint64_t stitchDiag[8] = {0, 0, 0, 0, 0, 0, 0, 0};
     uint32_t slotPercent = 95;
     uint32_t waveSlots = 256 * 4 * RESOLVE_WAVES_PER_SIMD;
     std::vector<Contig> contigs;
@@ -268,7 +276,7 @@
     const uint8_t *qdev = nullptr;
     uint32_t minLen = 0;
     bool batchValid = false;
-    uint64_t stats[6] = {0, 0, 0, 0, 0, 0};
+    uint64_t stats[9] = {0, 0, 0, 0, 0, 0, 0, 0, 0};
     bool prof = false;
     std::deque<ProfEvent> events;
     double profMs[SWSEM_K_COUNT] = {0};
```

Result: faster. 53.13, median of 6 (+1.8%).
